# AssafSinger94/dino-tracker

Measured on AMD Instinct MI355X. Metric: query-points*frames/s, higher is better.
Workload: dtype mixed: fp16 ViT operands (one per value), f16 conv operands in Delta-DINO, f16 candidates + f32 deciders in the tracker; f32 accumulate; 1 GPU; 854x480x90 synthetic video (model res 854x476, 67x121 tokens, C=384), 1024 grid queries; 1 video(s) per step over 1 GPU(s); features=vit, mode=single, track_method=mfma, anchor_pairs=92091, correlation_maps_per_video=8380350, rccl_ranks=1, parallelism=video-parallel x1

## Files before the change

### dino_tracker_amd/_lib.py

```python
from __future__ import annotations

import ctypes
import os

_HERE = os.path.dirname(os.path.abspath(__file__))
LIB_PATH = os.path.join(_HERE, "csrc", "libdtk.so")

c_int, c_float, c_void_p, c_size_t = ctypes.c_int, ctypes.c_float, ctypes.c_void_p, ctypes.c_size_t


class Geom(ctypes.Structure):
    _fields_ = [("T", ctypes.c_int32), ("C", ctypes.c_int32), ("ph", ctypes.c_int32), ("pw", ctypes.c_int32),
                ("video_h", ctypes.c_int32), ("video_w", ctypes.c_int32), ("patch", ctypes.c_int32),
                ("stride", ctypes.c_int32), ("radius", ctypes.c_float)]

    @property
    def HW(self) -> int:
        return self.ph * self.pw


def make_geom(T: int, C: int, video_h: int, video_w: int, patch: int = 14, stride: int = 7, radius: float = 35.0) -> Geom:
    ph = 1 + (video_h - patch) // stride
    pw = 1 + (video_w - patch) // stride
    return Geom(T, C, ph, pw, video_h, video_w, patch, stride, radius)
# ... 81 lines not shown
    "dtk_profile_collect": (c_int, []),
    "dtk_profile_name": (ctypes.c_char_p, [c_int]),
    "dtk_profile_ms": (ctypes.c_double, [c_int]),
    "dtk_profile_launches": (ctypes.c_longlong, [c_int]),
    "dtk_pack_features": (c_int, [c_void_p, c_void_p, c_void_p, c_int, c_int, c_int, c_void_p]),
    "dtk_unpack_features": (c_int, [c_void_p, c_void_p, c_int, c_int, c_int, c_void_p]),
    "dtk_feature_norms": (c_int, [c_void_p, c_void_p, c_int, c_int, c_int, c_void_p]),
    "dtk_vit_workspace_bytes": (c_size_t, [ctypes.POINTER(VitModel), c_int, c_int, c_int]),
    "dtk_vit_forward": (c_int, [ctypes.POINTER(VitModel), c_void_p, c_int, c_int, c_int, c_void_p, c_void_p, c_void_p,
                                c_void_p, c_size_t, c_void_p]),
    "dtk_vit_attention": (c_int, [c_void_p, c_void_p, c_void_p, c_void_p, c_int, c_int, c_int, c_int, c_int, c_void_p]),
    "dtk_vit_attention_split": (c_int, [c_void_p] * 8 + [c_int, c_int, c_int, c_int, c_int, c_void_p]),
    "dtk_vit_gemm": (c_int, [ctypes.POINTER(VitGemmArgs), c_void_p]),
    "dtk_vit_gemm_split": (c_int, [ctypes.POINTER(VitGemmArgs), c_void_p]),
    "dtk_delta_dino_packed_floats": (c_size_t, [c_int, c_int]),
    "dtk_delta_dino_pack": (c_int, [c_int, c_int, c_void_p, c_void_p, c_void_p, c_void_p, c_void_p, c_void_p, c_float,
                                    c_void_p, c_void_p]),
    "dtk_delta_dino_workspace_bytes": (c_size_t, [ctypes.POINTER(Geom)]),
    "dtk_delta_dino_refine": (c_int, [ctypes.POINTER(Geom), c_void_p, c_void_p, ctypes.POINTER(c_void_p), c_void_p,
                                      c_void_p, c_int, c_int, c_void_p, c_size_t, c_void_p]),
    "dtk_delta_dino_refine_mode": (c_int, [ctypes.POINTER(Geom), c_void_p, c_void_p, ctypes.POINTER(c_void_p), c_void_p,
                                           c_void_p, c_int, c_int, c_int, c_void_p, c_size_t, c_void_p]),
    "dtk_sample_points": (c_int, [ctypes.POINTER(Geom), c_void_p, c_void_p, c_void_p, c_void_p, c_void_p, c_int, c_void_p]),
    "dtk_sample_grid": (c_int, [c_void_p, c_int, c_int, c_int, c_int, c_void_p, c_void_p, c_int, c_void_p]),
    "dtk_normalized_conv2d": (c_int, [c_void_p, c_void_p, c_void_p, c_void_p, c_int, c_int, c_int, c_int, c_int, c_int,
                                      c_void_p]),
    "dtk_corr_maps": (c_int, [ctypes.POINTER(Geom), c_void_p, c_void_p, c_void_p, c_void_p, c_void_p, c_void_p, c_void_p,
                              c_int, c_int, c_void_p]),
    "dtk_head_prepare": (c_int, [c_void_p, c_void_p, c_void_p, c_void_p, c_void_p, c_void_p]),
    "dtk_head_forward": (c_int, [ctypes.POINTER(Geom), c_void_p, c_void_p, c_void_p, c_int, c_int, c_void_p]),
    "dtk_head_forward_train": (c_int, [ctypes.POINTER(Geom), c_void_p, c_void_p, c_void_p, c_void_p, c_int, c_int, c_void_p]),
    "dtk_conv_split_weight_halves": (c_size_t, [c_int, c_int]),
    "dtk_conv_split_pack": (c_int, [c_void_p, c_int, c_int, c_int, c_void_p, c_void_p, c_void_p]),
    "dtk_conv_split_input": (c_int, [c_void_p, c_int, c_int, c_int, c_int, c_int, c_void_p, c_void_p, c_void_p, c_void_p]),
    "dtk_conv_split_run": (c_int, [c_void_p, c_void_p, c_void_p, c_void_p, c_void_p, c_int, c_int, c_int, c_int, c_int, c_int,
                                   c_int, c_int, c_void_p]),
    "dtk_conv_split_output": (c_int, [c_void_p, c_int, c_int, c_int, c_int, c_int, c_int, c_void_p, c_void_p, c_void_p]),
    "dtk_conv_wgrad_split_workspace_bytes": (c_size_t, [c_int, c_int, c_int, c_int, c_int, c_int]),
    "dtk_conv_wgrad_split": (c_int, [c_void_p, c_void_p, c_void_p, c_int, c_int, c_int, c_int, c_int, c_int, c_int, c_void_p,
                                     c_int, c_void_p, c_size_t, c_void_p]),
    "dtk_gemm_nt_f32_indexed": (c_int, [c_void_p, c_void_p, c_void_p, c_int, c_int, c_int, ctypes.c_int64, ctypes.c_int64,
                                        ctypes.c_int64, c_int, ctypes.c_int64, ctypes.c_int64, ctypes.c_int64, c_int, c_int,
                                        c_void_p, c_void_p, c_void_p, c_void_p, c_void_p]),
    "dtk_contrastive_workspace_bytes": (c_size_t, [c_int, c_int, c_int, c_int]),
    "dtk_contrastive_forward": (c_int, [c_void_p, c_void_p, c_void_p, ctypes.c_float, c_int, c_int, c_int, c_int, c_int, c_void_p,
                                        c_void_p, c_void_p, c_void_p, c_void_p, c_void_p]),
    "dtk_contrastive_backward": (c_int, [c_void_p, c_void_p, c_void_p, ctypes.c_float, c_int, c_int, c_int, c_int, c_int, c_void_p,
                                         c_void_p, c_void_p, c_void_p, c_void_p, c_void_p, c_void_p, c_void_p, c_size_t, c_void_p]),
    "dtk_emb_reg_forward": (c_int, [c_void_p, c_void_p, c_int, c_int, c_int, c_void_p, c_void_p, c_void_p]),
    "dtk_sample_bilinear_forward": (c_int, [c_void_p, c_void_p, c_void_p, ctypes.c_int32, ctypes.c_int32, ctypes.c_int32, ctypes.c_int32, ctypes.c_int32, c_void_p]),
    "dtk_sample_bilinear_backward": (c_int, [c_void_p, c_void_p, c_void_p, ctypes.c_int32, ctypes.c_int32, ctypes.c_int32, ctypes.c_int32, ctypes.c_int32, c_void_p]),
    "dtk_pow2_scale": (c_int, [c_void_p, ctypes.c_int64, c_void_p, c_void_p, c_void_p]),
    "dtk_adam_step": (c_int, [ctypes.POINTER(AdamArgs), c_void_p]),
    "dtk_adam_scalars": (c_int, [ctypes.POINTER(AdamArgs), ctypes.POINTER(ctypes.c_float)]),
    "dtk_adam_step_dev": (c_int, [ctypes.POINTER(AdamArgs), c_void_p, c_void_p]),
    "dtk_emb_reg_backward": (c_int, [c_void_p, c_void_p, c_void_p, c_void_p, c_int, c_int, c_int, c_void_p, c_void_p]),
    "dtk_corr_window_backward": (c_int, [ctypes.POINTER(Geom), c_void_p, c_void_p, c_void_p, c_void_p, c_void_p, c_void_p, c_void_p,
                                         c_void_p, c_void_p, c_int, c_void_p]),
    "dtk_head_backward": (c_int, [ctypes.POINTER(Geom), c_void_p, c_void_p, c_void_p, c_void_p, c_void_p, c_void_p, c_int, c_int,
                                  c_void_p]),
    "dtk_track_workspace_bytes": (c_size_t, [ctypes.POINTER(Geom), c_int, ctypes.POINTER(TrackOpts)]),
    "dtk_track": (c_int, [ctypes.POINTER(Geom), c_void_p, c_void_p, c_void_p, c_void_p, c_void_p, c_void_p, c_void_p,
                          c_void_p, c_void_p, c_int, c_void_p, ctypes.POINTER(TrackOpts), ctypes.POINTER(TrackStats),
                          c_void_p, c_size_t, c_void_p]),
    "dtk_argmax_cells": (c_int, [ctypes.POINTER(Geom), c_void_p, c_void_p, c_void_p, c_void_p, c_void_p, c_void_p, c_void_p,
                                 c_void_p, c_int, c_int, c_void_p, c_size_t, c_void_p]),
    "dtk_bb_nms_workspace_bytes": (c_size_t, [ctypes.POINTER(Geom), c_int]),
    "dtk_bb_nms": (c_int, [ctypes.POINTER(Geom), c_void_p, c_void_p, c_void_p, c_void_p, c_void_p, c_float, c_float, c_int,
                           c_void_p, c_void_p, c_int, c_void_p, c_size_t, c_void_p]),
    "dtk_traj_start_fg": (c_int, [c_void_p, c_int, c_int, c_void_p, c_int, c_int, c_int, c_void_p, c_void_p, c_void_p]),
    "dtk_nearest_traj_workspace_bytes": (c_size_t, [c_int, c_int, c_int, c_int]),
    "dtk_nearest_traj": (c_int, [c_void_p, c_int, c_int, c_int, c_int, c_float, c_float, c_void_p, c_void_p, c_size_t, c_void_p]),
    "dtk_of_filter_keep": (c_int, [c_void_p, c_int, c_int, c_void_p, c_int, c_int, c_float, c_float, c_void_p, c_void_p,
                                   c_void_p, c_void_p, c_int, c_void_p, c_void_p, c_void_p]),
    "dtk_feat_f16_bytes": (c_size_t, [ctypes.POINTER(Geom)]),
    "dtk_make_feat_f16": (c_int, [ctypes.POINTER(Geom), c_void_p, c_void_p, c_void_p, c_void_p]),
    "dtk_traj_cos_sims": (c_int, [c_void_p, c_void_p, c_void_p, c_int, c_int, c_int, c_void_p]),
    "dtk_build_anchor_sources": (c_int, [c_void_p, c_float, c_int, c_int, c_void_p, c_void_p, c_void_p, c_void_p,
                                         c_void_p, c_void_p, c_void_p, c_void_p, c_void_p]),
    "dtk_occlusion": (c_int, [c_void_p, c_void_p, c_void_p, c_void_p, c_void_p, c_float, c_float, c_void_p, c_int,
                              c_int, c_void_p]),
    "dtk_build_anchor_sources_needed": (c_int, [c_void_p, c_float, c_float, c_int, c_int, c_void_p, c_void_p, c_void_p,
                                                c_void_p, c_void_p, c_void_p, c_void_p, c_void_p, c_void_p]),
    "dtk_occlusion_needed": (c_int, [c_void_p, c_void_p, c_void_p, c_void_p, c_void_p, c_float, c_float, c_void_p, c_int,
                                     c_int, c_void_p]),
    "dtk_tapvid_counts": (c_int, [c_void_p, c_void_p, c_void_p, c_void_p, c_void_p, c_float, c_float, c_float, c_float,
                                  c_int, c_int, c_int, c_void_p, c_void_p]),
    "dtk_badja_counts": (c_int, [c_void_p, c_void_p, c_void_p, c_void_p, c_int, c_float, c_float, c_int, c_int, c_int, c_int, c_int,
                                 c_void_p, c_void_p, c_void_p]),
    "dtk_blurpool_forward": (c_int, [c_void_p, c_void_p, ctypes.c_int64, c_int, c_int, c_void_p]),
    "dtk_blurpool_backward": (c_int, [c_void_p, c_void_p, ctypes.c_int64, c_int, c_int, c_void_p]),
    "dtk_gemm_nt_f32": (c_int, [c_void_p, c_void_p, c_void_p, c_int, c_int, c_int, ctypes.c_int64, ctypes.c_int64, ctypes.c_int64,
                                c_int, ctypes.c_int64, ctypes.c_int64, ctypes.c_int64, c_int, c_int, c_void_p, c_void_p, c_void_p]),
    "dtk_im2col": (c_int, [c_void_p, c_void_p, c_int, c_int, c_int, c_int, c_int, c_int, c_int, c_int, c_int, c_int,
                           ctypes.c_int64, c_void_p]),
    "dtk_col2im": (c_int, [c_void_p, c_void_p, c_int, c_int, c_int, c_int, c_int, c_int, c_int, c_int, c_int, c_void_p]),
    "dtk_transpose_f32": (c_int, [c_void_p, c_void_p, ctypes.c_int64, ctypes.c_int64, c_int, c_void_p]),
    "dtk_resample2d_forward": (c_int, [c_void_p, c_void_p, ctypes.c_int64, c_int, c_int, c_int, c_int, c_void_p, c_void_p, c_void_p,
                                       c_void_p, c_void_p]),
    "dtk_resample2d_backward": (c_int, [c_void_p, c_void_p, ctypes.c_int64, c_int, c_int, c_int, c_int, c_void_p, c_void_p,
                                        c_void_p, c_void_p, c_void_p]),
    "dtk_batchnorm_workspace_bytes": (c_size_t, [c_int]),
    "dtk_batchnorm_train_forward": (c_int, [c_void_p, c_void_p, c_void_p, c_void_p, c_void_p, c_void_p, c_float, c_float,
                                            c_int, c_void_p, c_void_p, c_void_p, c_int, c_int, c_int, c_void_p, c_size_t,
                                            c_void_p]),
    "dtk_batchnorm_train_backward": (c_int, [c_void_p, c_void_p, c_void_p, c_void_p, c_void_p, c_void_p, c_int, c_void_p,
                                             c_void_p, c_void_p, c_void_p, c_int, c_int, c_int, c_void_p, c_size_t, c_void_p]),
    "dtk_pca_moments_workspace_bytes": (c_size_t, [ctypes.c_int64, c_int, ctypes.c_int64]),
    "dtk_pca_moments": (c_int, [c_void_p, ctypes.c_int64, c_int, c_int, ctypes.c_int64, c_void_p, c_void_p, c_void_p, c_size_t,
                                c_void_p]),
    "dtk_pca_project_workspace_bytes": (c_size_t, [ctypes.c_int64]),
    "dtk_pca_project": (c_int, [c_void_p, ctypes.c_int64, c_int, c_int, c_void_p, c_int, c_void_p, c_void_p, c_void_p, c_size_t,
                                c_void_p]),
    "dtk_fg_mask": (c_int, [c_void_p, c_int, c_int, c_void_p, c_float, c_int, c_int, c_int, c_int, c_int, c_int, c_void_p, c_void_p,
                            c_void_p]),
    "dtk_flow_pack": (c_int, [c_void_p, c_void_p, c_int, c_int, c_int, c_void_p]),
    "dtk_flow_cycle_masks": (c_int, [c_void_p, c_void_p, c_int, c_int, c_int, c_float, c_void_p, c_void_p]),
    "dtk_flow_traj_workspace_bytes": (c_size_t, [c_int, c_int, c_int]),
    "dtk_flow_traj_start": (c_int, [c_void_p, c_void_p, c_void_p, c_void_p, c_int, c_int, c_int, c_int, c_float, c_int, c_void_p,
                                    c_void_p, c_int, c_float, c_void_p, c_void_p, c_size_t, c_void_p]),
    "dtk_flow_traj_emit": (c_int, [c_int, c_int, c_int, c_int, c_int, c_int, c_void_p, c_void_p, c_void_p, c_size_t, c_void_p]),
    "dtk_render_prim_count": (ctypes.c_int64, [c_int, c_int, c_int, c_int]),
    "dtk_render_group_bytes": (c_size_t, [ctypes.c_int64, ctypes.c_int64, c_int, c_int, c_int]),
    "dtk_render_prims": (c_int, [c_void_p, c_void_p, c_void_p, c_void_p, c_int, c_int, c_int, c_int, c_int, c_int, c_int, c_int,
                                 c_float, c_float, c_int, c_void_p, c_void_p]),
    "dtk_render_pred_gt_prims": (c_int, [c_void_p, c_void_p, c_void_p, c_void_p, c_void_p, c_int, c_int, c_int, c_int, c_int,
                                         c_int, c_int, c_void_p, c_void_p]),
    "dtk_render_tile_counts": (c_int, [c_void_p, ctypes.c_int64, c_int, c_int, c_int, c_void_p, c_void_p]),
    "dtk_render_tile_keys": (c_int, [c_void_p, c_void_p, ctypes.c_int64, c_int, c_int, c_int, ctypes.c_int64, c_void_p, c_void_p]),
    "dtk_render_blend": (c_int, [c_void_p, c_void_p, ctypes.c_int64, c_void_p, ctypes.c_int64, c_void_p, c_int, c_int, c_int,
                                 c_void_p, c_void_p, c_void_p]),
    "dtk_resize_workspace_bytes": (c_size_t, [c_int, c_int, c_int, c_int, c_int, c_int, c_int, c_int]),
    "dtk_resize_u8": (c_int, [c_void_p, c_int, c_int, c_int, c_int, c_int, c_int, c_void_p, c_void_p, c_int, c_void_p, c_void_p, c_int,
                              c_void_p, c_int, c_int, c_void_p, c_void_p, c_size_t, c_void_p]),
    "dtk_raft_conv_packed_halves": (c_size_t, [c_int, c_int, c_int, c_int]),
    "dtk_raft_conv_pack": (c_int, [c_void_p, c_int, c_int, c_int, c_int, c_float, c_void_p, c_void_p, c_void_p]),
    "dtk_raft_conv": (c_int, [ctypes.POINTER(RaftConvArgs), c_void_p]),
    "dtk_raft_instance_norm_workspace_bytes": (c_size_t, [c_int, c_int, c_int, c_int]),
    "dtk_raft_instance_norm": (c_int, [c_void_p, c_void_p, c_void_p, c_int, c_int, c_int, c_int, c_float, c_int, c_void_p, c_size_t,
                                       c_void_p]),
    "dtk_raft_pyramid_floats": (c_size_t, [c_int, c_int, c_int]),
    "dtk_raft_corr_pyramid": (c_int, [c_void_p, c_void_p, c_int, c_int, c_int, c_int, c_int, c_void_p, c_void_p]),
    "dtk_raft_lookup": (c_int, [c_void_p, c_void_p, ctypes.c_int64, c_int, c_int, c_int, c_void_p, ctypes.c_int64, c_void_p]),
    "dtk_raft_upsample": (c_int, [c_void_p, ctypes.c_int64, c_void_p, c_int, c_int, c_int, c_void_p, c_void_p]),
    "dtk_raft_workspace_bytes": (c_size_t, [c_int, c_int, c_int]),
    "dtk_raft_forward": (c_int, [ctypes.POINTER(RaftModel), c_void_p, c_void_p, c_int, c_int, c_int, c_int, c_int, c_void_p, c_void_p,
                                 c_size_t, c_void_p]),
}

_LIB = None


def lib() -> ctypes.CDLL:
    global _LIB
    if _LIB is None:
        if not os.path.isfile(LIB_PATH):
            raise RuntimeError(
                f"{LIB_PATH} is missing: build the HIP extension first (python -c 'import __graft_entry__ as g; "
                "g.build()' or make -C dino_tracker_amd/csrc). There is no CPU fallback for the hot path.")
        handle = ctypes.CDLL(LIB_PATH)
        for name, (res, args) in SIGNATURES.items():
            fn = getattr(handle, name)
            fn.restype = res
            fn.argtypes = args
        _LIB = handle
    return _LIB


# ... 4 lines not shown
```

### dino_tracker_amd/csrc/anchors.hip

```cpp
#include "common.h"

namespace {

__device__ __forceinline__ bool is_anchor(const float* cs, float th, int n, int T, int t) {
    return cs[(size_t)n * T + t] >= th;
}

__device__ __forceinline__ bool is_undecided(float c, float anchor_th, float cos_th) { return !(c >= anchor_th) && !(c < cos_th); }
__device__ __forceinline__ bool is_needed(float c, float anchor_th, float cos_th) { return c >= anchor_th || !(c < cos_th); }

__global__ __launch_bounds__(256) void query_need_kernel(const float* __restrict__ cs, float anchor_th, float cos_th, int N, int T,
                                                         int32_t* __restrict__ n_anchors, int32_t* __restrict__ need_w) {
    const int n = blockIdx.x * blockDim.x + threadIdx.x;
    if (n >= N) return;
    int anchors = 0, undecided = 0, needed = 0;
    for (int t = 0; t < T; ++t) {
        const float c = cs[(size_t)n * T + t];
        anchors += c >= anchor_th ? 1 : 0;
        undecided += is_undecided(c, anchor_th, cos_th) ? 1 : 0;
        needed += is_needed(c, anchor_th, cos_th) ? 1 : 0;
    }
    n_anchors[n] = anchors;
    need_w[n] = (anchors > 0 && undecided > 0) ? needed : 0;
}
// ... 89 lines not shown
}

__global__ void finalize_counts_kernel(const int32_t* __restrict__ pair_off, int N, int T, int32_t* __restrict__ counts) {
    if (threadIdx.x == 0 && blockIdx.x == 0) {
        counts[0] = pair_off[N];
        counts[1] = pair_off[N] * T;
    }
}

__global__ __launch_bounds__(256) void emit_sources_kernel(const float* __restrict__ cs, float th, int N, int T,
                                                           const int32_t* __restrict__ pair_off,
                                                           const int32_t* __restrict__ frame_off,
                                                           int32_t* __restrict__ pair_frame,
                                                           int32_t* __restrict__ src_row, int32_t* __restrict__ tgt,
                                                           int32_t* __restrict__ out_idx) {
    __shared__ int lds4[4];
    const int a = blockIdx.x;
    int carry = frame_off[a];
    for (int n0 = 0; n0 < N; n0 += 256) {
        const int n = n0 + threadIdx.x;
        const int flag = (n < N && is_anchor(cs, th, n, T, a)) ? 1 : 0;
        int total;
        const int incl = block_scan_incl(flag, lds4, &total);
        if (flag) {
            const int j = carry + incl - 1;
            int rank = 0;
            for (int t = 0; t < a; ++t) rank += is_anchor(cs, th, n, T, t) ? 1 : 0;
            const int p = pair_off[n] + rank;
            pair_frame[p] = a;
            const size_t mb = (size_t)j * T;
            for (int t = 0; t < T; ++t) {
                src_row[mb + t] = n * T + t;
                tgt[mb + t] = a;
                out_idx[mb + t] = p * T + t;
            }
        }
        carry += total;
    }
}

__global__ __launch_bounds__(256) void emit_needed_sources_kernel(const float* __restrict__ cs, float anchor_th, float cos_th,
                                                                  int N, int T, const int32_t* __restrict__ pair_off,
                                                                  const int32_t* __restrict__ frame_off,
                                                                  const int32_t* __restrict__ need_w,
                                                                  int32_t* __restrict__ pair_frame,
                                                                  int32_t* __restrict__ src_row, int32_t* __restrict__ tgt,
                                                                  int32_t* __restrict__ out_idx) {
    __shared__ int lds4[4];
    const int a = blockIdx.x;
    int carry = frame_off[a];
    for (int n0 = 0; n0 < N; n0 += 256) {
        const int n = n0 + threadIdx.x;
        const bool anchor = n < N && is_anchor(cs, anchor_th, n, T, a);
        const int weight = anchor ? need_w[n] : 0;
        int total;
        const int incl = block_scan_incl(weight, lds4, &total);
        if (anchor) {
            int rank = 0;
            for (int t = 0; t < a; ++t) rank += is_anchor(cs, anchor_th, n, T, t) ? 1 : 0;
            const int p = pair_off[n] + rank;
            pair_frame[p] = a;
            if (weight > 0) {
                int m = carry + incl - weight;
                for (int t = 0; t < T; ++t) {
                    if (!is_needed(cs[(size_t)n * T + t], anchor_th, cos_th)) continue;
                    src_row[m] = n * T + t;
                    tgt[m] = a;
                    out_idx[m] = p * T + t;
                    ++m;
                }
            }
        }
        carry += total;
    }
}

__device__ __forceinline__ float anchor_dist(const float* __restrict__ green, const float* __restrict__ tr, int p, int a,
                                             int T, int t) {
    const float dx = green[((size_t)p * T + t) * 2] - tr[2 * a];
    const float dy = green[((size_t)p * T + t) * 2 + 1] - tr[2 * a + 1];
    return sqrtf(__fadd_rn(__fmul_rn(dx, dx), __fmul_rn(dy, dy)));
}

template <bool PRUNED>
__global__ __launch_bounds__(256) void occlusion_kernel(const float* __restrict__ green,
                                                        const int32_t* __restrict__ pair_off,
                                                        const int32_t* __restrict__ pair_frame,
                                                        const float* __restrict__ traj, const float* __restrict__ cs,
                                                        float anchor_th, float cos_th, uint8_t* __restrict__ occ, int N,
                                                        int T) {
    extern __shared__ float smem_occ[];
    float* med = smem_occ;
    __shared__ float red[4];
    const int n = blockIdx.x;
    const int lane = threadIdx.x & 63, w = threadIdx.x >> 6;
    float* d = smem_occ + T + w * T;
    const int p0 = pair_off[n], A = pair_off[n + 1] - p0;
    const float* tr = traj + (size_t)n * T * 2;
    if (A <= 0) {
        for (int t = threadIdx.x; t < T; t += 256) occ[(size_t)n * T + t] = 1;
        return;
    }
    if constexpr (PRUNED) {
        int undecided = 0;
        for (int t = threadIdx.x; t < T; t += 256) undecided |= is_undecided(cs[(size_t)n * T + t], anchor_th, cos_th) ? 1 : 0;
        if (!__syncthreads_or(undecided)) {
            for (int t = threadIdx.x; t < T; t += 256) occ[(size_t)n * T + t] = cs[(size_t)n * T + t] < cos_th ? 1 : 0;
            return;
        }
    }
    const int want = (A - 1) / 2;
    for (int t = w; t < T; t += 4) {
        if constexpr (PRUNED)
            if (!is_needed(cs[(size_t)n * T + t], anchor_th, cos_th)) continue;
        for (int k = lane; k < A; k += WAVE) d[k] = anchor_dist(green, tr, p0 + k, pair_frame[p0 + k], T, t);
        __builtin_amdgcn_fence(__ATOMIC_RELEASE, "wavefront");
        __builtin_amdgcn_wave_barrier();
        for (int k = lane; k < A; k += WAVE) {
            const float dk = d[k];
            int rank = 0;
            for (int k2 = 0; k2 < A; ++k2) {
                const float d2 = d[k2];
                rank += (d2 < dk || (d2 == dk && k2 < k)) ? 1 : 0;
            }
            if (rank == want) med[t] = dk;
        }
        __builtin_amdgcn_fence(__ATOMIC_RELEASE, "wavefront");
        __builtin_amdgcn_wave_barrier();
    }
    __syncthreads();
    float tau = -INFINITY;
    for (int t = threadIdx.x; t < T; t += 256)
        if (cs[(size_t)n * T + t] >= anchor_th) tau = fmaxf(tau, med[t]);
    tau = wave_max(tau);
    if (lane == 0) red[w] = tau;
    __syncthreads();
    tau = fmaxf(fmaxf(red[0], red[1]), fmaxf(red[2], red[3]));
    for (int t = threadIdx.x; t < T; t += 256) {
        const float c = cs[(size_t)n * T + t];
        const bool far = (!PRUNED || is_needed(c, anchor_th, cos_th)) && med[t] > tau;
        occ[(size_t)n * T + t] = (far || c < cos_th) ? 1 : 0;
    }
}

}

extern "C" int dtk_build_anchor_sources(const float* cs, float anchor_th, int N, int T, int32_t* n_anchors,
                                        int32_t* pair_off, int32_t* pair_frame, int32_t* src_row, int32_t* tgt,
                                        int32_t* out_idx, int32_t* counts, int32_t* scratch, void* stream) {
    DTK_REQUIRE(cs && n_anchors && pair_off && pair_frame && src_row && tgt && out_idx && counts && scratch,
                "dtk_build_anchor_sources: null pointer");
    DTK_REQUIRE(N > 0 && T > 0 && (long long)N * T * T < 2147483647LL, "dtk_build_anchor_sources: N*T*T out of range");
    hipStream_t st = dtk_stream(stream);
    int32_t* frame_cnt = scratch;
    int32_t* frame_off = scratch + T;
    DTK_LAUNCH("anchor_count", anchor_count_kernel, dim3(dtk_cdiv(N, 256)), dim3(256), 0, st, cs, anchor_th, N, T, n_anchors);
    DTK_LAUNCH("exclusive_scan", exclusive_scan_kernel, dim3(1), dim3(256), 0, st, n_anchors, pair_off, N, counts + 2);
    DTK_LAUNCH("frame_count", frame_count_kernel, dim3(T), dim3(256), 0, st, cs, anchor_th, N, T, frame_cnt);
    DTK_LAUNCH("exclusive_scan", exclusive_scan_kernel, dim3(1), dim3(256), 0, st, frame_cnt, frame_off, T, (int32_t*)nullptr);
    DTK_LAUNCH("finalize_counts", finalize_counts_kernel, dim3(1), dim3(64), 0, st, pair_off, N, T, counts);
    DTK_LAUNCH("emit_sources", emit_sources_kernel, dim3(T), dim3(256), 0, st, cs, anchor_th, N, T, pair_off, frame_off,
                       pair_frame, src_row, tgt, out_idx);
    return DTK_OK;
}

extern "C" int dtk_occlusion(const float* green, const int32_t* pair_off, const int32_t* pair_frame, const float* traj,
                             const float* cs, float anchor_th, float cos_th, uint8_t* occ, int N, int T, void* stream) {
    DTK_REQUIRE(green && pair_off && pair_frame && traj && cs && occ && N >= 0 && T > 0, "dtk_occlusion: bad args");
    DTK_REQUIRE((size_t)5 * T * sizeof(float) <= 60 * 1024, "dtk_occlusion: T=%d too large", T);
    if (N == 0) return DTK_OK;
    DTK_LAUNCH("occlusion", occlusion_kernel<false>, dim3(N), dim3(256), (size_t)5 * T * sizeof(float), dtk_stream(stream), green,
                       pair_off, pair_frame, traj, cs, anchor_th, cos_th, occ, N, T);
    return DTK_OK;
}

extern "C" int dtk_build_anchor_sources_needed(const float* cs, float anchor_th, float cos_th, int N, int T, int32_t* n_anchors,
                                               int32_t* pair_off, int32_t* pair_frame, int32_t* src_row, int32_t* tgt,
                                               int32_t* out_idx, int32_t* counts, int32_t* scratch, void* stream) {
    DTK_REQUIRE(cs && n_anchors && pair_off && pair_frame && src_row && tgt && out_idx && counts && scratch,
                "dtk_build_anchor_sources_needed: null pointer");
    DTK_REQUIRE(N > 0 && T > 0 && (long long)N * T * T < 2147483647LL, "dtk_build_anchor_sources_needed: N*T*T out of range");
    hipStream_t st = dtk_stream(stream);
    int32_t* frame_cnt = scratch;
    int32_t* frame_off = scratch + T;
    int32_t* need_w = scratch + 2 * T + 2;
    DTK_LAUNCH("query_need", query_need_kernel, dim3(dtk_cdiv(N, 256)), dim3(256), 0, st, cs, anchor_th, cos_th, N, T, n_anchors,
               need_w);
    DTK_LAUNCH("exclusive_scan", exclusive_scan_kernel, dim3(1), dim3(256), 0, st, n_anchors, pair_off, N, counts + 2);
    DTK_LAUNCH("frame_weight", frame_weight_kernel, dim3(T), dim3(256), 0, st, cs, anchor_th, N, T, need_w, frame_cnt);
    DTK_LAUNCH("exclusive_scan", exclusive_scan_kernel, dim3(1), dim3(256), 0, st, frame_cnt, frame_off, T, (int32_t*)nullptr);
    DTK_LAUNCH("finalize_counts", finalize_needed_counts_kernel, dim3(1), dim3(256), 0, st, pair_off, frame_off, need_w, N, T,
               counts);
    DTK_LAUNCH("emit_sources", emit_needed_sources_kernel, dim3(T), dim3(256), 0, st, cs, anchor_th, cos_th, N, T, pair_off,
               frame_off, need_w, pair_frame, src_row, tgt, out_idx);
    return DTK_OK;
}

extern "C" int dtk_occlusion_needed(const float* green, const int32_t* pair_off, const int32_t* pair_frame, const float* traj,
                                    const float* cs, float anchor_th, float cos_th, uint8_t* occ, int N, int T, void* stream) {
    DTK_REQUIRE(green && pair_off && pair_frame && traj && cs && occ && N >= 0 && T > 0, "dtk_occlusion_needed: bad args");
    DTK_REQUIRE((size_t)5 * T * sizeof(float) <= 60 * 1024, "dtk_occlusion_needed: T=%d too large", T);
    if (N == 0) return DTK_OK;
    DTK_LAUNCH("occlusion", occlusion_kernel<true>, dim3(N), dim3(256), (size_t)5 * T * sizeof(float), dtk_stream(stream), green,
                       pair_off, pair_frame, traj, cs, anchor_th, cos_th, occ, N, T);
    return DTK_OK;
}


__global__ __launch_bounds__(256) void tapvid_counts_kernel(const float* __restrict__ pred, const uint8_t* __restrict__ pred_occ,
                                                            const float* __restrict__ gt, const uint8_t* __restrict__ gt_occ,
                                                            const int32_t* __restrict__ qframe, float spx, float spy,
                                                            float sgx, float sgy, int first_mode, int N, int T,
                                                            unsigned long long* __restrict__ counts) {
    const long long i = (long long)blockIdx.x * 256 + threadIdx.x;
    int c[18];
#pragma unroll
    for (int k = 0; k < 18; ++k) c[k] = 0;
    if (i < (long long)N * T) {
        const int n = (int)(i / T), t = (int)(i - (long long)n * T);
        const int qf = qframe[n];
        const bool ev = first_mode ? (t > qf) : (t != qf);
        if (ev) {
            const bool vis = gt_occ[i] == 0, pvis = pred_occ[i] == 0;
            const float dx = __fsub_rn(__fmul_rn(pred[2 * i], spx), __fmul_rn(gt[2 * i], sgx));
            const float dy = __fsub_rn(__fmul_rn(pred[2 * i + 1], spy), __fmul_rn(gt[2 * i + 1], sgy));
            const float d2 = __fadd_rn(__fmul_rn(dx, dx), __fmul_rn(dy, dy));
            c[0] = 1;
            c[1] = (pvis == vis);
            c[2] = vis;
#pragma unroll
            for (int k = 0; k < 5; ++k) {
                const float th = (float)(1 << k);
                const bool within = d2 < th * th;
                c[3 + 3 * k] = within && vis;
                c[4 + 3 * k] = within && vis && pvis;
                c[5 + 3 * k] = ((!vis) && pvis) || ((!within) && pvis);
            }
        }
    }
#pragma unroll
    for (int k = 0; k < 18; ++k) {
        const int s = wave_sum_i(c[k]);
        if ((threadIdx.x & 63) == 0 && s) atomicAdd(&counts[k], (unsigned long long)s);
    }
}

extern "C" int dtk_tapvid_counts(const float* pred_tracks, const uint8_t* pred_occluded, const float* gt_tracks,
                                 const uint8_t* gt_occluded, const int32_t* query_frame, float pred_scale_x,
                                 float pred_scale_y, float gt_scale_x, float gt_scale_y, int first_mode, int N, int T,
                                 unsigned long long* counts18, void* stream) {
    DTK_REQUIRE(counts18, "dtk_tapvid_counts: null pointer");
    DTK_REQUIRE(N >= 0 && T > 0, "dtk_tapvid_counts: bad sizes");
    hipStream_t st = dtk_stream(stream);
    DTK_HIP(hipMemsetAsync(counts18, 0, 18 * sizeof(unsigned long long), st));
    if (N == 0) return DTK_OK;
    DTK_REQUIRE(pred_tracks && pred_occluded && gt_tracks && gt_occluded && query_frame, "dtk_tapvid_counts: null pointer");
    DTK_LAUNCH("tapvid_counts", tapvid_counts_kernel, dim3(dtk_cdiv((long long)N * T, 256)), dim3(256), 0, st, pred_tracks,
               pred_occluded, gt_tracks, gt_occluded, query_frame, pred_scale_x, pred_scale_y, gt_scale_x, gt_scale_y,
               first_mode, N, T, counts18);
    return DTK_OK;
}


template <typename M>
__global__ __launch_bounds__(256) void badja_area_kernel(const M* __restrict__ seg, long long HW,
                                                         unsigned long long* __restrict__ areas) {
    const M* frame = seg + (size_t)blockIdx.y * HW;
    int c = 0;
    for (long long p = (long long)blockIdx.x * 256 + threadIdx.x; p < HW; p += (long long)gridDim.x * 256) c += frame[p] > (M)0;
    c = wave_sum_i(c);
    if ((threadIdx.x & 63) == 0 && c) atomicAdd(&areas[blockIdx.y], (unsigned long long)c);
}

__global__ __launch_bounds__(256) void badja_counts_kernel(const float* __restrict__ pred, const double* __restrict__ gt,
                                                           const uint8_t* __restrict__ gt_occ,
                                                           const unsigned long long* __restrict__ areas, float spx, float spy,
                                                           int N, int T, int T_seg, unsigned long long* __restrict__ counts) {
    const long long idx = (long long)blockIdx.x * 256 + threadIdx.x;
    const int per = T_seg - 1;
    int vis = 0, in_seg = 0, in_3px = 0;
    if (idx < (long long)N * per) {
        const int n = (int)(idx / per), t = 1 + (int)(idx - (long long)n * per);
        const size_t at = (size_t)n * T + t;
        if (gt_occ[at] == 0) {
            const float thr = __fmul_rn(0.2f, __fsqrt_rn((float)areas[t]));
            const double dx = __dsub_rn((double)__fmul_rn(pred[2 * at], spx), gt[2 * at]);
            const double dy = __dsub_rn((double)__fmul_rn(pred[2 * at + 1], spy), gt[2 * at + 1]);
// ... 43 lines not shown
```

### dino_tracker_amd/csrc/track_exact.hip

```cpp
#include <limits.h>
#include "common.h"
#include "head_common.h"

namespace {

constexpr int TM = 64, TN = 64, TK = 16;
constexpr int HR = 6;
constexpr int HR_LARGE = 2;

__global__ void head_prepare_kernel(const float* __restrict__ w1, const float* __restrict__ b1,
                                    const float* __restrict__ w2, const float* __restrict__ b2,
                                    float* __restrict__ head) {
    const int ch = threadIdx.x;
    if (ch >= DTK_HEAD_HIDDEN) return;
    float s1 = 0.f, s2 = 0.f;
    for (int t = 0; t < 9; ++t) {
        s1 += w1[ch * 9 + t];
        s2 += w2[ch * 9 + t];
    }
    auto fix = [](float s) {
        if (fabsf(s) < 1e-8f) s = (s > 0.f ? 1.f : (s < 0.f ? -1.f : 0.f)) * 1e-8f;
        return s;
    };
    s1 = fix(s1);
    s2 = fix(s2);
    for (int t = 0; t < 9; ++t) {
        head[ch * 9 + t] = w1[ch * 9 + t] / s1;
        head[144 + 16 + ch * 9 + t] = w2[ch * 9 + t] / s2;
    }
    head[144 + ch] = b1[ch];
    if (ch == 0) head[144 + 16 + 144] = b2[0];
}

__global__ __launch_bounds__(256) void row_norms_kernel(const float* __restrict__ emb,
                                                        const int32_t* __restrict__ src_row,
                                                        float* __restrict__ snorm, int m0, int count, int M,
                                                        const int32_t* __restrict__ dM, int C) {
    const int i = blockIdx.x * 4 + (threadIdx.x >> 6);
    if (i >= count) return;
    const int lane = threadIdx.x & 63;
    const int m = m0 + i;
    float s = 0.f;
    if (m < dtk_active(M, dM)) {
        const float* p = emb + (size_t)(src_row ? src_row[m] : m) * C;
        for (int c = lane * 4; c < C; c += 256) {
            const float4 v = *reinterpret_cast<const float4*>(p + c);
            s += v.x * v.x + v.y * v.y + v.z * v.z + v.w * v.w;
        }
        s = wave_sum(s);
    }
    if (lane == 0) snorm[i] = sqrtf(s);
}

__global__ __launch_bounds__(256) void corr_exact_kernel(dtk_geom g, const float* __restrict__ feat,
                                                         const float* __restrict__ norms,
                                                         const float* __restrict__ emb,
                                                         const int32_t* __restrict__ src_row,
                                                         const int32_t* __restrict__ tgt,
                                                         const float* __restrict__ snorm, float* __restrict__ maps,
                                                         int m0, int count, int M, const int32_t* __restrict__ dM,
                                                         int HWs, int relu) {
    __shared__ __attribute__((aligned(16))) float As[TK][TM + 4];
    __shared__ __attribute__((aligned(16))) float Bs[TK][TN + 4];
    __shared__ int s_tgt[TM];
    __shared__ int s_row[TM];
    __shared__ int s_fr[2];
    const int HW = g.ph * g.pw;
    const int active = min(dtk_active(M, dM), m0 + count);
    const int tile_m0 = m0 + blockIdx.y * TM;
    if (tile_m0 >= active) return;
    const int cell0 = blockIdx.x * TN;
    const int tid = threadIdx.x;
    if (tid < TM) {
        const int m = tile_m0 + tid;
        const bool ok = m < active;
        int f = ok ? tgt[m] : -1;
        if (ok) f = min(max(f, 0), g.T - 1);
        s_tgt[tid] = f;
        s_row[tid] = ok ? (src_row ? src_row[m] : m) : (src_row ? src_row[tile_m0] : tile_m0);
        int lo = ok ? f : INT_MAX, hi = f;
#pragma unroll
        for (int o = 32; o > 0; o >>= 1) {
            lo = min(lo, __shfl_xor(lo, o, WAVE));
            hi = max(hi, __shfl_xor(hi, o, WAVE));
        }
        if (tid == 0) {
            s_fr[0] = lo;
            s_fr[1] = hi;
        }
    }
    __syncthreads();
    const int fmin = s_fr[0], fmax = s_fr[1];
    const int ty = tid >> 4, tx = tid & 15;
    const int lr = tid >> 2, lk = (tid & 3) * 4;
    const float* arow = emb + (size_t)s_row[lr] * g.C;
    const int lcell = cell0 + lr;
    for (int f = fmin; f <= fmax; ++f) {
        bool mine = false;
#pragma unroll
        for (int i = 0; i < 4; ++i) mine |= (s_tgt[ty * 4 + i] == f);
        if (!__syncthreads_or(mine)) continue;
        const float* brow = feat + ((size_t)f * HW + min(lcell, HW - 1)) * g.C;
        float acc[4][4];
#pragma unroll
        for (int i = 0; i < 4; ++i)
#pragma unroll
            for (int j = 0; j < 4; ++j) acc[i][j] = 0.f;
        for (int k0 = 0; k0 < g.C; k0 += TK) {
            float4 a = make_float4(0.f, 0.f, 0.f, 0.f), b = a;
            if (k0 + lk < g.C) {
                a = *reinterpret_cast<const float4*>(arow + k0 + lk);
                if (lcell < HW) b = *reinterpret_cast<const float4*>(brow + k0 + lk);
            }
            As[lk + 0][lr] = a.x; As[lk + 1][lr] = a.y; As[lk + 2][lr] = a.z; As[lk + 3][lr] = a.w;
            Bs[lk + 0][lr] = b.x; Bs[lk + 1][lr] = b.y; Bs[lk + 2][lr] = b.z; Bs[lk + 3][lr] = b.w;
            __syncthreads();
#pragma unroll
            for (int kk = 0; kk < TK; ++kk) {
                const float4 av = *reinterpret_cast<const float4*>(&As[kk][ty * 4]);
                const float4 bv = *reinterpret_cast<const float4*>(&Bs[kk][tx * 4]);
                const float aa[4] = {av.x, av.y, av.z, av.w}, bb[4] = {bv.x, bv.y, bv.z, bv.w};
#pragma unroll
                for (int i = 0; i < 4; ++i)
#pragma unroll
                    for (int j = 0; j < 4; ++j) acc[i][j] = fmaf(aa[i], bb[j], acc[i][j]);
            }
            __syncthreads();
        }
#pragma unroll
        for (int i = 0; i < 4; ++i) {
            const int r = ty * 4 + i;
            if (s_tgt[r] != f) continue;
            const int ml = tile_m0 - m0 + r;
            const float sn = snorm[ml];
#pragma unroll
            for (int j = 0; j < 4; ++j) {
                const int cell = cell0 + tx * 4 + j;
                if (cell < HW) {
                    const float den = fmaxf(sn * norms[(size_t)f * HW + cell], 1e-8f);
                    const float rho = acc[i][j] / den;
                    maps[(size_t)ml * HWs + cell] = relu ? fmaxf(rho, 0.f) : rho;
                }
            }
        }
    }
}

__device__ __forceinline__ float block_max(float v, float* red) {
    v = wave_max(v);
    __syncthreads();
    if ((threadIdx.x & 63) == 0) red[threadIdx.x >> 6] = v;
    __syncthreads();
    return fmaxf(fmaxf(red[0], red[1]), fmaxf(red[2], red[3]));
}
__device__ __forceinline__ float block_sum(float v, float* red) {
    v = wave_sum(v);
    __syncthreads();
    if ((threadIdx.x & 63) == 0) red[threadIdx.x >> 6] = v;
    __syncthreads();
    return (red[0] + red[1]) + (red[2] + red[3]);
}

}

namespace {

template <bool LARGE>
__global__ __launch_bounds__(256) void head_exact_kernel(dtk_geom g, const float* __restrict__ head,
                                                         const float* __restrict__ maps, int HWs,
                                                         const int32_t* __restrict__ out_idx,
                                                         float* __restrict__ out_xy, int m0, int count, int M,
                                                         const int32_t* __restrict__ dM, int normalized,
                                                         float* __restrict__ stats) {
    extern __shared__ __attribute__((aligned(16))) float smem[];
    const int HW = g.ph * g.pw, pw = g.pw, ph = g.ph;
    const int HWp = (HW + 3) & ~3;
    constexpr int HRK = LARGE ? HR_LARGE : HR;
    float* sz = LARGE ? smem : smem + HWp;
    float* sh = sz + HWp;
    float* red = sh + DTK_HEAD_HIDDEN * (HRK + 2) * pw;
    int* redi = reinterpret_cast<int*>(red + 8);
    const int i = blockIdx.x;
    const int m = m0 + i;
    if (i >= count || m >= dtk_active(M, dM)) return;
    const int tid = threadIdx.x;
    const float* map = maps + (size_t)i * HWs;
    const float* sx = map;
    if constexpr (!LARGE) {
        for (int c = tid; c < HW; c += 256) smem[c] = map[c];
        sx = smem;
    }
    __syncthreads();

    float best = -1.f;
    int bi = INT_MAX;
    for (int c = tid; c < HW; c += 256) {
        const float v = sx[c];
        if (v > best) { best = v; bi = c; }
    }
#pragma unroll
    for (int o = 32; o > 0; o >>= 1) {
        const float ov = __shfl_xor(best, o, WAVE);
        const int oi = __shfl_xor(bi, o, WAVE);
        if (ov > best || (ov == best && oi < bi)) { best = ov; bi = oi; }
    }
    if ((tid & 63) == 0) { red[tid >> 6] = best; redi[tid >> 6] = bi; }
    __syncthreads();
    best = red[0]; bi = redi[0];
#pragma unroll
    for (int w = 1; w < 4; ++w)
        if (red[w] > best || (red[w] == best && redi[w] < bi)) { best = red[w]; bi = redi[w]; }
    const int kstar = bi;
    __syncthreads();

    const float* w1 = head;
    const float* b1 = head + 144;
    const float* w2 = head + 160;
    const float b2 = head[304];
    const int ring = HRK + 2;
    for (int r0 = 0; r0 < ph; r0 += HRK) {
        const int nout = min(HRK, ph - r0);
        for (int idx = tid; idx < (nout + 2) * pw; idx += 256) {
            const int hr = idx / pw, c = idx - hr * pw;
// ... 81 lines not shown
    for (int o = 32; o > 0; o >>= 1) {
        const float ov = __shfl_xor(best, o, WAVE);
        const int oi = __shfl_xor(bi, o, WAVE);
        if (ov > best || (ov == best && oi < bi)) { best = ov; bi = oi; }
    }
    if ((tid & 63) == 0) { red[tid >> 6] = best; redi[tid >> 6] = bi; }
    __syncthreads();
    if (tid == 0) {
        best = red[0]; bi = redi[0];
        for (int w = 1; w < 4; ++w)
            if (red[w] > best || (red[w] == best && redi[w] < bi)) { best = red[w]; bi = redi[w]; }
        const int oi = out_idx ? out_idx[m0 + i] : m0 + i;
        arg_cell[oi] = bi;
        arg_cos[oi] = best;
    }
}

extern "C" int dtk_head_prepare(const float* w1, const float* b1, const float* w2, const float* b2, float* head,
                                void* stream) {
    DTK_REQUIRE(w1 && b1 && w2 && b2 && head, "dtk_head_prepare: null pointer");
    DTK_LAUNCH("head_prepare", head_prepare_kernel, dim3(1), dim3(64), 0, dtk_stream(stream), w1, b1, w2, b2, head);
    return DTK_OK;
}

extern "C" int dtk_head_forward(const dtk_geom* g, const float* head, const float* maps, float* out_xy, int B,
                                int normalized, void* stream);

static inline int exact_hws(const dtk_geom* g) { return (g->ph * g->pw + 63) & ~63; }
static inline size_t exact_head_lds(const dtk_geom* g, bool large) {
    const int HWp = (g->ph * g->pw + 3) & ~3;
    return sizeof(float) * (size_t)((large ? 1 : 2) * HWp + DTK_HEAD_HIDDEN * ((large ? HR_LARGE : HR) + 2) * g->pw + 16);
}
constexpr size_t EXACT_LDS_MAX = 160 * 1024;
static int launch_head_exact(const char* who, const char* name, const dtk_geom* g, const float* head, const float* maps, int HWs,
                             const int32_t* out_idx, float* out_xy, int m0, int cnt, int M, const int32_t* dM, int normalized,
                             float* stats, hipStream_t st) {
    const bool large = exact_head_lds(g, false) > EXACT_LDS_MAX;
    const size_t lds = exact_head_lds(g, large);
    DTK_REQUIRE(lds <= EXACT_LDS_MAX, "%s: token grid %dx%d needs %zu B of LDS (> 160 KiB)", who, g->ph, g->pw, lds);
    if (large) {
        DTK_HIP(hipFuncSetAttribute(reinterpret_cast<const void*>(head_exact_kernel<true>),
                                    hipFuncAttributeMaxDynamicSharedMemorySize, (int)lds));
        DTK_LAUNCH(name, head_exact_kernel<true>, dim3(cnt), dim3(256), lds, st, *g, head, maps, HWs, out_idx, out_xy, m0, cnt, M,
                   dM, normalized, stats);
    } else {
        DTK_HIP(hipFuncSetAttribute(reinterpret_cast<const void*>(head_exact_kernel<false>),
                                    hipFuncAttributeMaxDynamicSharedMemorySize, (int)lds));
        DTK_LAUNCH(name, head_exact_kernel<false>, dim3(cnt), dim3(256), lds, st, *g, head, maps, HWs, out_idx, out_xy, m0, cnt, M,
                   dM, normalized, stats);
    }
    return DTK_OK;
}
bool dtk_track_exact_fits(const dtk_geom* g) { return exact_head_lds(g, true) <= EXACT_LDS_MAX; }
constexpr int EXACT_CHUNK = 4096;

size_t dtk_track_exact_workspace_bytes(const dtk_geom* g, int M) {
    const int chunk = M < EXACT_CHUNK ? (M < 64 ? 64 : M) : EXACT_CHUNK;
    return (size_t)chunk * (exact_hws(g) + 1) * sizeof(float);
}

int dtk_track_exact(const dtk_geom* g, const float* feat, const float* norms, const float* head, const float* emb,
                    const int32_t* src_row, const int32_t* tgt, const int32_t* out_idx, float* out_xy, int M,
                    const int32_t* dM, int normalized, void* workspace, size_t workspace_bytes, void* stream) {
    DTK_REQUIRE(g->C % TK == 0, "dtk_track(exact): C=%d must be a multiple of %d", g->C, TK);
    const int HWs = exact_hws(g);
    DTK_REQUIRE(dtk_track_exact_fits(g), "dtk_track(exact): token grid %dx%d needs %zu B of LDS (> 160 KiB)", g->ph, g->pw,
                exact_head_lds(g, true));
    long long chunk = (long long)(workspace_bytes / ((size_t)(HWs + 1) * sizeof(float)));
    if (chunk > M) chunk = M;
    if (chunk > 65535LL * TM) chunk = 65535LL * TM;
    if (chunk < 1) {
        dtk_set_error("dtk_track(exact): workspace of %zu B holds no map (need %zu B per source)", workspace_bytes,
                      (size_t)(HWs + 1) * sizeof(float));
        return DTK_E_WORKSPACE;
    }
    hipStream_t st = dtk_stream(stream);
    float* maps = reinterpret_cast<float*>(workspace);
    float* snorm = maps + (size_t)chunk * HWs;
    const int HW = g->ph * g->pw;
    for (long long m0 = 0; m0 < M; m0 += chunk) {
        const int cnt = (int)((M - m0) < chunk ? (M - m0) : chunk);
        DTK_LAUNCH("row_norms", row_norms_kernel, dim3(dtk_cdiv(cnt, 4)), dim3(256), 0, st, emb, src_row, snorm, (int)m0,
                           cnt, M, dM, g->C);
        DTK_LAUNCH("corr_exact", corr_exact_kernel, dim3(dtk_cdiv(HW, TN), dtk_cdiv(cnt, TM)), dim3(256), 0, st, *g, feat,
                           norms, emb, src_row, tgt, snorm, maps, (int)m0, cnt, M, dM, HWs, 1);
        const int rc = launch_head_exact("dtk_track(exact)", "head_exact", g, head, maps, HWs, out_idx, out_xy, (int)m0, cnt, M, dM,
                                         normalized, nullptr, st);
        if (rc) return rc;
    }
    return DTK_OK;
}

extern "C" int dtk_head_forward(const dtk_geom* g, const float* head, const float* maps, float* out_xy, int B,
                                int normalized, void* stream) {
    DTK_REQUIRE(g && head && maps && out_xy && B >= 0, "dtk_head_forward: null pointer");
    DTK_REQUIRE(g->ph > 0 && g->pw > 0 && g->stride > 0 && g->patch > 0, "dtk_head_forward: bad geometry");
    if (B == 0) return DTK_OK;
    return launch_head_exact("dtk_head_forward", "head_exact", g, head, maps, g->ph * g->pw, nullptr, out_xy, 0, B, B, nullptr,
                             normalized, nullptr, dtk_stream(stream));
}

namespace {

constexpr int HB_RD = 5, HB_WX = 2 * HB_RD + 5, HB_WH = 2 * HB_RD + 3, HB_WZ = 2 * HB_RD + 1;

__global__ __launch_bounds__(256) void head_backward_kernel(dtk_geom g, const float* __restrict__ head,
                                                            const float* __restrict__ maps, const float* __restrict__ stats,
                                                            const float* __restrict__ gout, float* __restrict__ dmaps,
                                                            float* __restrict__ dhead, int B, int normalized) {
    constexpr int NH = HB_WH * HB_WH, NZ = HB_WZ * HB_WZ, XP = HB_WX + 1;
    __shared__ float s_x[4][HB_WX * XP];
    __shared__ float s_h[4][DTK_HEAD_HIDDEN * NH];
    __shared__ unsigned char s_m[4][DTK_HEAD_HIDDEN * NH];
    __shared__ float s_z[4][NZ], s_dz[4][NZ];
    const int lane = threadIdx.x & 63, w = threadIdx.x >> 6;
    const int b = blockIdx.x * 4 + w;
    if (b >= B) return;
    const int ph = g.ph, pw = g.pw, HW = ph * pw;
    const float* st = stats + 4 * (size_t)b;
    const int kstar = __float_as_int(st[0]);
    const float zmax = st[1], Z = st[2];
    const int kr = kstar / pw, kc = kstar % pw;
    const float* map = maps + (size_t)b * HW;
    const float* w1 = head;
    const float* b1 = head + 144;
    const float* w2 = head + 160;
    const float b2 = head[304];
    float* sx = s_x[w];
    float* sh = s_h[w];
    unsigned char* sm = s_m[w];
    float* sz = s_z[w];
    float* sdz = s_dz[w];
    auto wsync = [] {
        __builtin_amdgcn_fence(__ATOMIC_RELEASE, "wavefront");
        __builtin_amdgcn_wave_barrier();
        __builtin_amdgcn_fence(__ATOMIC_ACQUIRE, "wavefront");
    };
    for (int i = lane; i < HB_WX * HB_WX; i += WAVE) {
        const int jr = i / HB_WX, jc = i - jr * HB_WX;
        const int r = kr - (HB_RD + 2) + jr, c = kc - (HB_RD + 2) + jc;
        sx[jr * XP + jc] = (r >= 0 && r < ph && c >= 0 && c < pw) ? map[r * pw + c] : 0.f;
    }
    wsync();
    for (int i = lane; i < NH; i += WAVE) {
        const int hy = i / HB_WH, hx = i - hy * HB_WH;
        const int r = kr - (HB_RD + 1) + hy, c = kc - (HB_RD + 1) + hx;
        const bool in = r >= 0 && r < ph && c >= 0 && c < pw;
        float x9[9];
#pragma unroll
        for (int dy = 0; dy < 3; ++dy)
#pragma unroll
            for (int dx = 0; dx < 3; ++dx) x9[dy * 3 + dx] = sx[(hy + dy) * XP + hx + dx];
#pragma unroll
        for (int ch = 0; ch < DTK_HEAD_HIDDEN; ++ch) {
            float a = 0.f;
#pragma unroll
            for (int t = 0; t < 9; ++t) a = fmaf(w1[ch * 9 + t], x9[t], a);
            a += b1[ch];
            const bool pos = in && a > 0.f;
            sh[ch * NH + i] = pos ? a : 0.f;
            sm[ch * NH + i] = pos ? 1 : 0;
        }
    }
    wsync();
    for (int i = lane; i < NZ; i += WAVE) {
        const int zy = i / HB_WZ, zx = i - zy * HB_WZ;
        float a = 0.f;
// ... 151 lines not shown
    const float* fbase = feat + (size_t)f * HW * C;
    float* dbase = dfeat + (size_t)f * HW * C;
    const float* mp = maps + (size_t)b * HW;
    const float* dm = dmaps + (size_t)b * HW;
    const int r0 = max(kr - (HB_RD + 2), 0), r1 = min(kr + (HB_RD + 2), ph - 1);
    const int c0 = max(kc - (HB_RD + 2), 0), c1 = min(kc + (HB_RD + 2), pw - 1);
    for (int r = r0 + w; r <= r1; r += 4)
        for (int c = c0; c <= c1; ++c) {
            const int cell = r * pw + c;
            const float gk = dm[cell], rho = mp[cell];
            if (gk == 0.f || !(rho > 0.f)) continue;
            const float fn = norms[(size_t)f * HW + cell];
            const float den = sn * fn;
            const bool clamped = !(den > 1e-8f);
            const float inv_den = clamped ? 1e8f : 1.f / den;
            const float a_s = clamped ? 0.f : rho * inv_ss;
            const float a_f = clamped ? 0.f : rho / (fn * fn);
            const float* fp = fbase + (size_t)cell * C;
            float* dp = dbase + (size_t)cell * C;
#pragma unroll
            for (int j = 0; j < MAXJ; ++j) {
                const int ch = j * WAVE + lane;
                if (j < nj && ch < C) {
                    const float fv = fp[ch];
                    ds[j] += gk * (fv * inv_den - a_s * s[j]);
                    atomicAdd(dp + ch, gk * (s[j] * inv_den - a_f * fv));
                }
            }
        }
#pragma unroll
    for (int j = 0; j < MAXJ; ++j) s_ds[w][j * WAVE + lane] = ds[j];
    __syncthreads();
    for (int c = threadIdx.x; c < C; c += 256) demb[(size_t)b * C + c] = (s_ds[0][c] + s_ds[1][c]) + (s_ds[2][c] + s_ds[3][c]);
}

}

extern "C" int dtk_corr_window_backward(const dtk_geom* g, const float* feat, const float* norms, const float* emb,
                                        const int32_t* tgt, const float* maps, const float* dmaps, const float* stats,
                                        float* demb, float* dfeat, int B, void* stream) {
    DTK_REQUIRE(g && feat && norms && emb && tgt && maps && dmaps && stats && demb && dfeat && B >= 0,
                "dtk_corr_window_backward: null pointer");
    DTK_REQUIRE(g->C > 0 && g->C <= 1024, "dtk_corr_window_backward: C=%d outside 1..1024", g->C);
    DTK_REQUIRE(g->radius / (float)g->stride <= (float)HB_RD, "dtk_corr_window_backward: radius / stride > %d", HB_RD);
    if (B == 0) return DTK_OK;
    DTK_LAUNCH("train_corr_bwd", corr_window_backward_kernel, dim3(B), dim3(256), 0, dtk_stream(stream), *g, feat,
               norms, emb, tgt, maps, dmaps, stats, demb, dfeat, B);
    return DTK_OK;
}

extern "C" int dtk_head_forward_train(const dtk_geom* g, const float* head, const float* maps, float* out_xy, float* stats, int B,
                                      int normalized, void* stream) {
    DTK_REQUIRE(g && head && maps && out_xy && stats && B >= 0, "dtk_head_forward_train: null pointer");
    DTK_REQUIRE(g->ph > 0 && g->pw > 0 && g->stride > 0 && g->patch > 0, "dtk_head_forward_train: bad geometry");
    if (B == 0) return DTK_OK;
    return launch_head_exact("dtk_head_forward_train", "train_head_fwd", g, head, maps, g->ph * g->pw, nullptr, out_xy, 0, B, B,
                             nullptr, normalized, stats, dtk_stream(stream));
}

extern "C" int dtk_head_backward(const dtk_geom* g, const float* head, const float* maps, const float* stats, const float* grad_out,
                                 float* dmaps, float* dhead_partial, int B, int normalized, void* stream) {
    DTK_REQUIRE(g && head && maps && stats && grad_out && dmaps && dhead_partial && B >= 0, "dtk_head_backward: null pointer");
    DTK_REQUIRE(g->stride > 0 && g->radius / (float)g->stride <= (float)HB_RD,
                "dtk_head_backward: disk radius %g px exceeds %d cells of stride %d", (double)g->radius, HB_RD, g->stride);
    if (B == 0) return DTK_OK;
    DTK_LAUNCH("train_head_bwd", head_backward_kernel, dim3(dtk_cdiv(B, 4)), dim3(256), 0, dtk_stream(stream), *g, head, maps,
               stats, grad_out, dmaps, dhead_partial, B, normalized);
    return DTK_OK;
}

extern "C" int dtk_corr_maps(const dtk_geom* g, const float* feat, const float* norms, const float* emb,
                             const int32_t* src_row, const int32_t* tgt, float* maps, float* snorm_scratch, int M,
                             int relu, void* stream) {
    DTK_REQUIRE(g && feat && norms && emb && tgt && maps && snorm_scratch, "dtk_corr_maps: null pointer");
    DTK_REQUIRE(g->T > 0 && g->ph > 0 && g->pw > 0 && g->C > 0 && g->C % TK == 0, "dtk_corr_maps: bad geometry (C %% %d)", TK);
    DTK_REQUIRE(M >= 0, "dtk_corr_maps: negative M");
    const int HW = g->ph * g->pw;
    hipStream_t st = dtk_stream(stream);
    const long long step = 65535LL * TM;
    for (long long m0 = 0; m0 < M; m0 += step) {
        const int cnt = (int)((M - m0) < step ? (M - m0) : step);
        DTK_LAUNCH("row_norms", row_norms_kernel, dim3(dtk_cdiv(cnt, 4)), dim3(256), 0, st, emb, src_row, snorm_scratch + m0,
                   (int)m0, cnt, M, (const int32_t*)nullptr, g->C);
        DTK_LAUNCH("corr_exact", corr_exact_kernel, dim3(dtk_cdiv(HW, TN), dtk_cdiv(cnt, TM)), dim3(256), 0, st, *g, feat,
                   norms, emb, src_row, tgt, snorm_scratch + m0, maps + (size_t)m0 * HW, (int)m0, cnt, M,
                   (const int32_t*)nullptr, HW, relu);
    }
    return DTK_OK;
}

int dtk_argmax_exact(const dtk_geom* g, const float* feat, const float* norms, const float* emb, const int32_t* src_row,
                     const int32_t* tgt, const int32_t* out_idx, int32_t* arg_cell, float* arg_cos, int M, void* workspace,
                     size_t workspace_bytes, void* stream) {
    DTK_REQUIRE(g->C % TK == 0, "dtk_argmax_cells(exact): C=%d must be a multiple of %d", g->C, TK);
    const int HWs = exact_hws(g), HW = g->ph * g->pw;
    long long chunk = (long long)(workspace_bytes / ((size_t)(HWs + 1) * sizeof(float)));
    if (chunk > M) chunk = M;
    if (chunk > 65535LL * TM) chunk = 65535LL * TM;
    if (chunk < 1) {
        dtk_set_error("dtk_argmax_cells(exact): workspace of %zu B holds no map", workspace_bytes);
        return DTK_E_WORKSPACE;
    }
    hipStream_t st = dtk_stream(stream);
    float* maps = reinterpret_cast<float*>(workspace);
    float* snorm = maps + (size_t)chunk * HWs;
    for (long long m0 = 0; m0 < M; m0 += chunk) {
        const int cnt = (int)((M - m0) < chunk ? (M - m0) : chunk);
        DTK_LAUNCH("row_norms", row_norms_kernel, dim3(dtk_cdiv(cnt, 4)), dim3(256), 0, st, emb, src_row, snorm, (int)m0, cnt, M,
                   (const int32_t*)nullptr, g->C);
        DTK_LAUNCH("corr_exact", corr_exact_kernel, dim3(dtk_cdiv(HW, TN), dtk_cdiv(cnt, TM)), dim3(256), 0, st, *g, feat, norms,
                   emb, src_row, tgt, snorm, maps, (int)m0, cnt, M, (const int32_t*)nullptr, HWs, 0);
        DTK_LAUNCH("argmax_exact", argmax_exact_kernel, dim3(cnt), dim3(256), 0, st, maps, HW, HWs, out_idx, arg_cell, arg_cos,
                   (int)m0, cnt);
    }
    return DTK_OK;
}

namespace {

constexpr int NMS_VPT = 40;

__device__ __forceinline__ unsigned order_key(float v) {
    const unsigned b = __float_as_uint(v);
    return (b & 0x80000000u) ? ~b : (b | 0x80000000u);
}

__global__ __launch_bounds__(256) void bb_nms_kernel(dtk_geom g, const float* __restrict__ maps, int HWs, float box_half,
                                                     float iou_thresh, int topk, float* __restrict__ peak_affs,
                                                     float* __restrict__ r_out, int m0, int count) {
    __shared__ float red[4];
    __shared__ int redi[4];
    __shared__ int s_cnt;
    const int i = blockIdx.x;
    if (i >= count) return;
    const int tid = threadIdx.x, HW = g.ph * g.pw;
    const float* map = maps + (size_t)i * HWs;
    float v[NMS_VPT];
    float best = -INFINITY;
    int bi = INT_MAX;
#pragma unroll
    for (int j = 0; j < NMS_VPT; ++j) {
        const int c = tid + 256 * j;
        v[j] = c < HW ? map[c] : -INFINITY;
        if (c < HW && v[j] > best) { best = v[j]; bi = c; }
    }
#pragma unroll
    for (int o = 32; o > 0; o >>= 1) {
        const float ov = __shfl_xor(best, o, WAVE);
        const int oi = __shfl_xor(bi, o, WAVE);
        if (ov > best || (ov == best && oi < bi)) { best = ov; bi = oi; }
    }
    if ((tid & 63) == 0) { red[tid >> 6] = best; redi[tid >> 6] = bi; }
    __syncthreads();
    best = red[0]; bi = redi[0];
#pragma unroll
    for (int w = 1; w < 4; ++w)
        if (red[w] > best || (red[w] == best && redi[w] < bi)) { best = red[w]; bi = redi[w]; }
    unsigned K = 0;
    for (int bit = 31; bit >= 0; --bit) {
        const unsigned cand = K | (1u << bit);
        int c = 0;
#pragma unroll
        for (int j = 0; j < NMS_VPT; ++j) c += (tid + 256 * j < HW && order_key(v[j]) >= cand) ? 1 : 0;
        c = wave_sum_i(c);
        __syncthreads();
        if (tid == 0) s_cnt = 0;
        __syncthreads();
        if ((tid & 63) == 0) atomicAdd(&s_cnt, c);
        __syncthreads();
        if (s_cnt >= topk) K = cand;
    }
    const float half = (float)(g.patch / 2), st = (float)g.stride;
    const float pcx = half + st * (float)(bi % g.pw), pcy = half + st * (float)(bi / g.pw);
    const float px1 = pcx - box_half, px2 = pcx + box_half, py1 = pcy - box_half, py2 = pcy + box_half;
    const float parea = (px2 - px1) * (py2 - py1);
    float b = -INFINITY;
    int nsupp = 0;
#pragma unroll
    for (int j = 0; j < NMS_VPT; ++j) {
        const int c = tid + 256 * j;
        if (c < HW && c != bi && order_key(v[j]) >= K) {
            const float cx = half + st * (float)(c % g.pw), cy = half + st * (float)(c / g.pw);
            const float x1 = cx - box_half, x2 = cx + box_half, y1 = cy - box_half, y2 = cy + box_half;
            const float iw = fmaxf(fminf(x2, px2) - fmaxf(x1, px1), 0.f), ih = fmaxf(fminf(y2, py2) - fmaxf(y1, py1), 0.f);
            const float inter = iw * ih;
            const float iou = inter / (parea + (x2 - x1) * (y2 - y1) - inter);
            if (iou > iou_thresh) ++nsupp;
            else b = fmaxf(b, v[j]);
        }
    }
    b = wave_max(b);
    nsupp = wave_sum_i(nsupp);
    __syncthreads();
    if ((tid & 63) == 0) { red[tid >> 6] = b; redi[tid >> 6] = nsupp; }
    __syncthreads();
    if (tid == 0) {
        b = fmaxf(fmaxf(red[0], red[1]), fmaxf(red[2], red[3]));
        nsupp = redi[0] + redi[1] + redi[2] + redi[3];
        float c4[4] = {best, b, nsupp >= 1 ? 0.f : -INFINITY, nsupp >= 2 ? 0.f : -INFINITY};
        float t1 = -INFINITY, t2 = -INFINITY;
#pragma unroll
        for (int q = 0; q < 4; ++q) {
            if (c4[q] > t1) { t2 = t1; t1 = c4[q]; }
            else if (c4[q] > t2) t2 = c4[q];
        }
        peak_affs[2 * (size_t)(m0 + i)] = t1;
        peak_affs[2 * (size_t)(m0 + i) + 1] = t2;
        r_out[m0 + i] = t2 / t1;
    }
}

}

extern "C" size_t dtk_bb_nms_workspace_bytes(const dtk_geom* g, int M) { return dtk_track_exact_workspace_bytes(g, M); }

extern "C" int dtk_bb_nms(const dtk_geom* g, const float* feat, const float* norms, const float* emb, const int32_t* src_row,
                          const int32_t* tgt, float box_size, float iou_thresh, int topk, float* peak_affs, float* r, int M,
                          void* workspace, size_t workspace_bytes, void* stream) {
    DTK_REQUIRE(g && feat && norms && emb && tgt && peak_affs && r && workspace, "dtk_bb_nms: null pointer");
    DTK_REQUIRE(M >= 0, "dtk_bb_nms: negative M");
    if (M == 0) return DTK_OK;
    DTK_REQUIRE(g->C % TK == 0, "dtk_bb_nms: C=%d must be a multiple of %d", g->C, TK);
    const int HWs = exact_hws(g), HW = g->ph * g->pw;
    DTK_REQUIRE(HW <= 256 * NMS_VPT, "dtk_bb_nms: %d cells per frame (max %d)", HW, 256 * NMS_VPT);
    DTK_REQUIRE(topk >= 2 && topk <= HW, "dtk_bb_nms: topk=%d must be in [2, %d] (torch.topk)", topk, HW);
    long long chunk = (long long)(workspace_bytes / ((size_t)(HWs + 1) * sizeof(float)));
    if (chunk > M) chunk = M;
    if (chunk > 65535LL * TM) chunk = 65535LL * TM;
    if (chunk < 1) {
        dtk_set_error("dtk_bb_nms: workspace of %zu B holds no map", workspace_bytes);
        return DTK_E_WORKSPACE;
    }
    hipStream_t st = dtk_stream(stream);
    float* maps = reinterpret_cast<float*>(workspace);
    float* snorm = maps + (size_t)chunk * HWs;
    for (long long m0 = 0; m0 < M; m0 += chunk) {
        const int cnt = (int)((M - m0) < chunk ? (M - m0) : chunk);
        DTK_LAUNCH("row_norms", row_norms_kernel, dim3(dtk_cdiv(cnt, 4)), dim3(256), 0, st, emb, src_row, snorm, (int)m0, cnt, M,
                   (const int32_t*)nullptr, g->C);
        DTK_LAUNCH("corr_exact", corr_exact_kernel, dim3(dtk_cdiv(HW, TN), dtk_cdiv(cnt, TM)), dim3(256), 0, st, *g, feat, norms,
                   emb, src_row, tgt, snorm, maps, (int)m0, cnt, M, (const int32_t*)nullptr, HWs, 0);
        DTK_LAUNCH("bb_nms", bb_nms_kernel, dim3(cnt), dim3(256), 0, st, *g, maps, HWs, box_size, iou_thresh, topk, peak_affs, r,
                   (int)m0, cnt);
    }
    return DTK_OK;
}
```

### dino_tracker_amd/csrc/track_mfma.hip

```cpp
#include <limits.h>
#include <stdlib.h>
#include <type_traits>
#include "common.h"
#include "head_common.h"

int dtk_track_exact(const dtk_geom* g, const float* feat, const float* norms, const float* head, const float* emb,
                    const int32_t* src_row, const int32_t* tgt, const int32_t* out_idx, float* out_xy, int M,
                    const int32_t* dM, int normalized, void* workspace, size_t workspace_bytes, void* stream);
size_t dtk_track_exact_workspace_bytes(const dtk_geom* g, int M);
bool dtk_track_exact_fits(const dtk_geom* g);

namespace {

typedef _Float16 half_t;
typedef _Float16 h2 __attribute__((ext_vector_type(2)));
typedef _Float16 h8 __attribute__((ext_vector_type(8)));
typedef float f4 __attribute__((ext_vector_type(4)));

constexpr float FSCALE = 32.f;
constexpr float INV_SCALE2 = 1.f / 1024.f;
constexpr float EPS_C = 3e-3f;
constexpr int KC = 10;
constexpr int CM = 64, CN = 128, CK = 32;
constexpr int NB_MAX = 1024;
constexpr int RD = 5;
constexpr int MFMA_CHUNK = 16384;
constexpr int MFMA_SUPER = 4194304;

struct Rec {
    float amax;
    int ncand;
    int cand[KC];
    float zmax, Z;
};

__host__ __device__ inline int pw_pad(int pw) { return (pw + CN - 1) / CN * CN; }
__host__ __device__ inline int map_xw(int pw) { return pw_pad(pw) + 16; }
__host__ __device__ inline int hw_pad(int ph, int pw) { return ph * pw_pad(pw); }

__global__ __launch_bounds__(256) void feat16_kernel(const float* __restrict__ feat, const float* __restrict__ norms,
                                                     half_t* __restrict__ f16, int T, int ph, int pw, int PWP, int C) {
    const long long cell = (long long)blockIdx.x * 4 + (threadIdx.x >> 6);
    const int HWp = ph * PWP, HW = ph * pw;
    if (cell >= (long long)T * HWp) return;
    const int lane = threadIdx.x & 63;
    const int t = (int)(cell / HWp), pc = (int)(cell % HWp);
    const int r = pc / PWP, c = pc - r * PWP;
    half_t* o = f16 + cell * C;
    if (c >= pw) {
        for (int k = lane * 8; k < C; k += 512) *reinterpret_cast<uint4*>(o + k) = make_uint4(0, 0, 0, 0);
        return;
    }
    const float* p = feat + ((size_t)t * HW + r * pw + c) * C;
    const float nrm = norms[(size_t)t * HW + r * pw + c];
    const float sc = nrm > 1e-30f ? FSCALE / nrm : 0.f;
    for (int k = lane * 8; k < C; k += 512) {
        const float4 a = *reinterpret_cast<const float4*>(p + k), b = *reinterpret_cast<const float4*>(p + k + 4);
        h8 v = {(half_t)(a.x * sc), (half_t)(a.y * sc), (half_t)(a.z * sc), (half_t)(a.w * sc),
                (half_t)(b.x * sc), (half_t)(b.y * sc), (half_t)(b.z * sc), (half_t)(b.w * sc)};
        *reinterpret_cast<h8*>(o + k) = v;
    }
}

__host__ __device__ inline bool peaks_wide_ok(int C) { return C == 768 || C == 1024; }

constexpr float RC_SCALE_MAX = 32.f;
__host__ __device__ inline size_t split_planes_offset(const dtk_geom* g) {
    return ((size_t)g->T * hw_pad(g->ph, g->pw) * g->C * 2 + 255) / 256 * 256;
}
__host__ __device__ inline bool has_split_planes(const dtk_geom* g) {
    return g->C == 384 && (long long)g->T * g->ph * g->pw * g->C * 4 < (1LL << 32);
}
__host__ __device__ inline size_t rc_scale_offset(const dtk_geom* g) {
    const size_t unit = (size_t)g->T * hw_pad(g->ph, g->pw) * g->C * 2;
    const size_t end = has_split_planes(g) ? split_planes_offset(g) + (size_t)g->T * g->ph * g->pw * g->C * 4 : unit;
    return (end + 255) / 256 * 256;
}
__global__ __launch_bounds__(256) void rcscale_max_kernel(const float* __restrict__ norms, long long n, unsigned* __restrict__ slot) {
    float m = 0.f;
    for (long long i = (long long)blockIdx.x * 256 + threadIdx.x; i < n; i += (long long)gridDim.x * 256) {
        const float v = norms[i];
        m = fmaxf(m, v == v ? v : 3.0e38f);
    }
    m = wave_max(m);
    if ((threadIdx.x & 63) == 0) atomicMax(slot + 1, __float_as_uint(m));
}
__global__ void rcscale_final_kernel(unsigned* __restrict__ slot) {
    const float m = __uint_as_float(slot[1]);
    float sc = RC_SCALE_MAX;
    while (sc > 0x1p-40f && m * sc > 16384.f) sc *= 0.5f;
    reinterpret_cast<float*>(slot)[0] = sc;
}
__global__ __launch_bounds__(256) void featsplit_kernel(const float* __restrict__ feat, half_t* __restrict__ fs,
                                                        long long n8, const float* __restrict__ rc_scale) {
    const long long i = (long long)blockIdx.x * 256 + threadIdx.x;
    if (i >= n8) return;
    const float RC_SCALE = *rc_scale;
    const float4 a = *reinterpret_cast<const float4*>(feat + i * 8), b = *reinterpret_cast<const float4*>(feat + i * 8 + 4);
    const float x[8] = {a.x, a.y, a.z, a.w, b.x, b.y, b.z, b.w};
    h8 hi, lo;
#pragma unroll
    for (int e = 0; e < 8; ++e) {
        const float xs = x[e] * RC_SCALE;
        hi[e] = (half_t)xs;
        lo[e] = (half_t)(xs - (float)hi[e]);
    }
    const long long chunk = i >> 2;
    const int piece = (int)(i & 3);
    *reinterpret_cast<h8*>(fs + chunk * 64 + piece * 8) = hi;
    *reinterpret_cast<h8*>(fs + chunk * 64 + 32 + piece * 8) = lo;
}

__global__ __launch_bounds__(256) void src16_kernel(const float* __restrict__ emb, const int32_t* __restrict__ src_row,
                                                    half_t* __restrict__ s16, int m0, int count, int M,
                                                    const int32_t* __restrict__ dM, int C, float scale,
                                                    float* __restrict__ rown) {
    const int i = blockIdx.x * 4 + (threadIdx.x >> 6);
    if (i >= count) return;
    const int lane = threadIdx.x & 63;
    const int m = m0 + i;
    half_t* o = s16 + (size_t)i * C;
    if (m >= dtk_active(M, dM)) {
        for (int k = lane * 8; k < C; k += 512) *reinterpret_cast<uint4*>(o + k) = make_uint4(0, 0, 0, 0);
        return;
    }
    const float* p = emb + (size_t)(src_row ? src_row[m] : m) * C;
    float s = 0.f;
    for (int k = lane * 4; k < C; k += 256) {
        const float4 v = *reinterpret_cast<const float4*>(p + k);
        s += v.x * v.x + v.y * v.y + v.z * v.z + v.w * v.w;
    }
    s = sqrtf(wave_sum(s));
    if (rown && lane == 0) rown[i] = s;
    const float sc = s > 1e-30f ? scale / s : 0.f;
    for (int k = lane * 8; k < C; k += 512) {
        const float4 a = *reinterpret_cast<const float4*>(p + k), b = *reinterpret_cast<const float4*>(p + k + 4);
        h8 v = {(half_t)(a.x * sc), (half_t)(a.y * sc), (half_t)(a.z * sc), (half_t)(a.w * sc),
                (half_t)(b.x * sc), (half_t)(b.y * sc), (half_t)(b.z * sc), (half_t)(b.w * sc)};
        *reinterpret_cast<h8*>(o + k) = v;
    }
}

__device__ __forceinline__ int swz(int row, int piece) {
    const int f = (0x1230 >> (((row >> 2) & 3) * 4)) & 3;
    return row * 4 + (piece ^ f);
}

struct TileRec {
    float v1, v2;
    uint32_t idx;
};

template <bool PEAKS>
__global__ __launch_bounds__(256) void corr16_tiled_kernel(dtk_geom g, const half_t* __restrict__ f16,
                                                     const half_t* __restrict__ s16, const int32_t* __restrict__ tgt,
                                                     half_t* __restrict__ maps, TileRec* __restrict__ trec, int m0,
                                                     int count, int M, const int32_t* __restrict__ dM, int HWp, int MP,
                                                     int dbg) {
    __shared__ uint4 smem_ab[2 * (CM + CN) * 4];
    uint4 (*As)[CM * 4] = reinterpret_cast<uint4 (*)[CM * 4]>(smem_ab);
    uint4 (*Bs)[CN * 4] = reinterpret_cast<uint4 (*)[CN * 4]>(smem_ab + 2 * CM * 4);
    half_t* Ts = reinterpret_cast<half_t*>(smem_ab);
    constexpr int TP16 = CN + 8;
    __shared__ int s_tgt[CM];
    __shared__ int s_fr[2];
    const int active = min(dtk_active(M, dM), m0 + count);
    const int NT = HWp / CN, MT = (count + CM - 1) / CM;
    int bx, by;
    {
        const int L = blockIdx.x, xcd = L & 7, k = L >> 3;
        const int mt_per = (MT + 7) >> 3;
        const int per_panel = mt_per * 8;
        const int p = k / per_panel, rem = k - p * per_panel;
        by = (rem >> 3) * 8 + xcd;
        bx = p * 8 + (rem & 7);
        if (by >= MT || bx >= NT) return;
    }
    const int tile_m0 = m0 + by * CM;
    if (tile_m0 >= active) return;
    const int cell0 = bx * CN;
    const int tid = threadIdx.x, lane = tid & 63, w = tid >> 6;
    if (tid < CM) {
        const int m = tile_m0 + tid;
        const bool ok = m < active;
        int f = ok ? min(max(tgt[m], 0), g.T - 1) : -1;
        s_tgt[tid] = f;
        int lo = ok ? f : INT_MAX, hi = f;
#pragma unroll
        for (int o = 32; o > 0; o >>= 1) {
            lo = min(lo, __shfl_xor(lo, o, WAVE));
            hi = max(hi, __shfl_xor(hi, o, WAVE));
        }
        if (tid == 0) { s_fr[0] = lo; s_fr[1] = hi; }
// ... 1606 lines not shown
            redo.out_idx[slot] = oi;
        } else {
            out_xy[2 * (size_t)oi] = s_out[w][0];
            out_xy[2 * (size_t)oi + 1] = s_out[w][1];
        }
    }
}

struct MfmaLayout {
    size_t s16, maps, rec, wpk, kstar, xwin, snorm, rown, perm, hist, off, cursor, bsum, nvalid, redo_cnt, redo_lists, exact, total;
    int HWk, nkeys, nblocks, cap;
    size_t unc_lists, trec;
    int MP;
    int chunk;
    int super;
    int HWp;
};

MfmaLayout mfma_layout(const dtk_geom* g, int M, int round_sources) {
    MfmaLayout L;
    L.chunk = M < MFMA_CHUNK ? ((M + CM - 1) / CM * CM) : MFMA_CHUNK;
    const int round = round_sources > 0 ? (round_sources + 255) / 256 * 256 : MFMA_SUPER;
    L.super = M < round ? ((M + CM - 1) / CM * CM) : round;
    if (L.chunk > L.super) L.chunk = L.super;
    L.HWp = hw_pad(g->ph, g->pw);
    auto al = [](size_t x) { return (x + 255) & ~(size_t)255; };
    size_t off = 0;
    L.s16 = off; off = al(off + (size_t)L.super * g->C * 2);
    L.MP = ((g->ph + 2) * map_xw(g->pw) + 32 + 7) & ~7;
    L.maps = off; off = al(off + (size_t)L.chunk * L.MP * 2);
    L.rec = off; off = al(off + (size_t)L.super * sizeof(Rec));
    L.trec = off; off = al(off + (size_t)L.chunk * (L.HWp / CN) * sizeof(TileRec));
    L.wpk = off; off = al(off + 256 * 4);
    L.kstar = off; off = al(off + (size_t)L.super * 4);
    L.xwin = off; off = al(off + (size_t)L.super * WX * WX * 4);
    L.HWk = (g->ph + 7) / 8 * 8 * g->pw;
    L.nkeys = g->T * L.HWk;
    L.nblocks = (L.nkeys + SCAN_PER_BLOCK - 1) / SCAN_PER_BLOCK;
    L.snorm = off; off = al(off + (size_t)L.super * 4);
    L.rown = off; off = al(off + (size_t)L.super * 4);
    L.perm = off; off = al(off + (size_t)L.super * 4);
    L.hist = off; off = al(off + (size_t)L.nkeys * 4);
    L.cursor = off; off = al(off + (size_t)L.nkeys * 4);
    L.off = off; off = al(off + (size_t)(L.nkeys + 1) * 4);
    L.bsum = off; off = al(off + (size_t)(L.nblocks + 1) * 4);
    L.nvalid = off; off = al(off + 16);
    L.cap = (M + CM - 1) / CM * CM;
    L.redo_cnt = off; off = al(off + 16);
    L.redo_lists = off; off = al(off + (size_t)3 * L.cap * 4);
    L.unc_lists = off; off = al(off + (size_t)3 * L.cap * 4);
    L.exact = off;
    const int redo_rows = L.super < 65536 ? L.super : 65536;
    L.total = off + (size_t)redo_rows * (((size_t)g->ph * g->pw + 63) / 64 * 64 + 1) * sizeof(float);
    return L;
}

}

size_t dtk_track_mfma_workspace_bytes(const dtk_geom* g, int M, int round_sources) {
    return mfma_layout(g, M, round_sources).total;
}

#ifdef DTK_DEV
extern "C" int dtk_debug_counters(unsigned long long* out4) {
    unsigned long long z[4] = {0, 0, 0, 0};
    DTK_HIP(hipMemcpyFromSymbol(out4, HIP_SYMBOL(g_dbg), sizeof(z)));
    DTK_HIP(hipMemcpyToSymbol(HIP_SYMBOL(g_dbg), z, sizeof(z)));
    return DTK_OK;
}
#endif

extern "C" size_t dtk_feat_f16_bytes(const dtk_geom* g) {
    if (!g || g->T <= 0 || g->C <= 0) return 0;
    const size_t unit = (size_t)g->T * hw_pad(g->ph, g->pw) * g->C * 2;
    (void)unit;
    return rc_scale_offset(g) + 256;
}

extern "C" int dtk_make_feat_f16(const dtk_geom* g, const float* feat, const float* norms, void* feat_f16, void* stream) {
    DTK_REQUIRE(g && feat && norms && feat_f16, "dtk_make_feat_f16: null pointer");
    DTK_REQUIRE(g->C % CK == 0, "dtk_make_feat_f16: C=%d must be a multiple of %d for the MFMA path", g->C, CK);
    const int HWp = hw_pad(g->ph, g->pw);
    const long long cells = (long long)g->T * HWp;
    DTK_LAUNCH("feat16", feat16_kernel, dim3(dtk_cdiv(cells, 4)), dim3(256), 0, dtk_stream(stream), feat, norms,
               reinterpret_cast<half_t*>(feat_f16), g->T, g->ph, g->pw, pw_pad(g->pw), g->C);
    unsigned* slot = reinterpret_cast<unsigned*>(reinterpret_cast<unsigned char*>(feat_f16) + rc_scale_offset(g));
    DTK_HIP(dtk_zero_async(slot, 256, dtk_stream(stream)));
    {
        const long long nn = (long long)g->T * g->ph * g->pw;
        const int blocks = (int)(dtk_cdiv(nn, 256) < 512 ? dtk_cdiv(nn, 256) : 512);
        DTK_LAUNCH("rcscale", rcscale_max_kernel, dim3(blocks), dim3(256), 0, dtk_stream(stream), norms, nn, slot);
        DTK_LAUNCH("rcscale", rcscale_final_kernel, dim3(1), dim3(1), 0, dtk_stream(stream), slot);
    }
    if (has_split_planes(g)) {
        const long long n8 = (long long)g->T * g->ph * g->pw * g->C / 8;
        DTK_LAUNCH("featsplit", featsplit_kernel, dim3(dtk_cdiv(n8, 256)), dim3(256), 0, dtk_stream(stream), feat,
                   reinterpret_cast<half_t*>(reinterpret_cast<unsigned char*>(feat_f16) + split_planes_offset(g)), n8,
                   reinterpret_cast<const float*>(slot));
    }
    return DTK_OK;
}

namespace {

struct SrcLists {
    const int32_t *src_row, *tgt, *out_idx;
};

int mfma_phase(const dtk_geom* g, const MfmaLayout& L, unsigned char* ws, const float* feat, const float* norms,
               const half_t* f16, const float* head, const float* emb, SrcLists in, float* out_xy, int count,
               int normalized, bool fast, Redo redo, Redo uncert, size_t lds_head, hipStream_t st, int dbg,
               int32_t* arg_cell = nullptr, float* arg_cos = nullptr, bool row_table = false) {
    half_t* s16 = reinterpret_cast<half_t*>(ws + L.s16);
    half_t* maps = reinterpret_cast<half_t*>(ws + L.maps);
    Rec* rec = reinterpret_cast<Rec*>(ws + L.rec);
    uint32_t* wpk = reinterpret_cast<uint32_t*>(ws + L.wpk);
    int32_t* kstar = reinterpret_cast<int32_t*>(ws + L.kstar);
    float* xwin = reinterpret_cast<float*>(ws + L.xwin);
    int32_t* hist = reinterpret_cast<int32_t*>(ws + L.hist);
    int32_t* cursor = reinterpret_cast<int32_t*>(ws + L.cursor);
    int32_t* koff = reinterpret_cast<int32_t*>(ws + L.off);
    int32_t* bsum = reinterpret_cast<int32_t*>(ws + L.bsum);
    int32_t* nvalid = reinterpret_cast<int32_t*>(ws + L.nvalid);
    float* snorm = reinterpret_cast<float*>(ws + L.snorm);
    int32_t* perm = reinterpret_cast<int32_t*>(ws + L.perm);
    const int32_t* nodm = nullptr;
    const int M = count;
    for (long long s0 = 0; s0 < M; s0 += L.super) {
        const int scnt = (int)((M - s0) < L.super ? (M - s0) : L.super);
        const int pk_cb = DTK_DBG(dbg, 65536) ? 2 : PK_CB, pk_cells = 32 * pk_cb;
        const bool peaks_shape = L.HWp / pk_cells <= (1 << (PK_IDX_BITS - (pk_cb > 1 ? 5 : 4))) &&
                                 L.HWp % pk_cells == 0 && pw_pad(g->pw) % pk_cells == 0 && !DTK_DBG(dbg, 2048) &&
                                 (long long)g->T * L.HWp * g->C * 2 < (1LL << 32);
        const bool peaks_wide = fast && peaks_wide_ok(g->C) && pk_cb == 1 && peaks_shape;
        const bool peaks = (fast && g->C == 384 && peaks_shape) || peaks_wide;
        DTK_HIP(hipMemsetAsync(ws + L.hist, 0, L.cursor + (size_t)L.nkeys * 4 - L.hist, st));
        if (peaks) {
            const int32_t* row_of = row_table ? in.src_row : nullptr;
            if (!row_of)
                DTK_LAUNCH("src16", src16_kernel, dim3(dtk_cdiv(scnt, 4)), dim3(256), 0, st, emb, in.src_row, s16, (int)s0, scnt, M,
                           nodm, g->C, PK_SRC_SCALE, (float*)nullptr);
            const dim3 pgrid(dtk_cdiv(scnt, peaks_wide ? PKW_SRC : PK_SRC));
            const bool fuse_done = row_table && arg_cell == nullptr && !DTK_DBG(dbg, 2);
            const PeaksDone pdone = fuse_done ? PeaksDone{kstar, snorm, hist, reinterpret_cast<const float*>(ws + L.rown), L.HWk}
                                              : PeaksDone{nullptr, nullptr, nullptr, nullptr, 0};
#define DTK_PEAKS(V, CBV)                                                                                                    \
    do {                                                                                                                     \
        static const hipError_t attr_ = hipFuncSetAttribute(reinterpret_cast<const void*>(&corr_peaks_kernel<24, V, CBV>),  \
                                                            hipFuncAttributeMaxDynamicSharedMemorySize,                      \
                                                            (int)peaks_lds_bytes(CBV));                                      \
        DTK_HIP(attr_);                                                                                                      \
        DTK_LAUNCH("corr_peaks", (corr_peaks_kernel<24, V, CBV>), pgrid, dim3(256), peaks_lds_bytes(CBV), st, *g, f16, s16,  \
                   in.tgt, rec, (int)s0, scnt, L.HWp, row_of, pdone);                                                        \
    } while (0)
#define DTK_PEAKS_WIDE(KSHV)                                                                                                  \
    do {                                                                                                                     \
        static const hipError_t attr_ = hipFuncSetAttribute(reinterpret_cast<const void*>(&corr_peaks_wide_kernel<KSHV>),   \
                                                            hipFuncAttributeMaxDynamicSharedMemorySize,                      \
                                                            (int)peaks_wide_lds_bytes(32 * KSHV));                           \
        DTK_HIP(attr_);                                                                                                      \
        DTK_LAUNCH("corr_peaks", (corr_peaks_wide_kernel<KSHV>), pgrid, dim3(256), peaks_wide_lds_bytes(32 * KSHV), st, *g,  \
                   f16, s16, in.tgt, rec, (int)s0, scnt, L.HWp, row_of, pdone);                                              \
    } while (0)
            if (peaks_wide) {
                if (g->C == 1024) DTK_PEAKS_WIDE(32);
                else DTK_PEAKS_WIDE(24);
            } else
#ifdef DTK_DEV
            if (pk_cb == 2) {
                switch ((dbg >> 13) & 7) {
                    case 0: DTK_PEAKS(0, 2); break;
                    case 1: DTK_PEAKS(1, 2); break;
                    case 2: DTK_PEAKS(2, 2); break;
                    case 4: DTK_PEAKS(4, 2); break;
                    default: DTK_PEAKS(7, 2); break;
                }
            } else {
                switch ((dbg >> 13) & 7) {
                    case 0: DTK_PEAKS(0, PK_CB); break;
                    case 1: DTK_PEAKS(1, PK_CB); break;
                    case 2: DTK_PEAKS(2, PK_CB); break;
// ... 184 lines not shown
```

### dino_tracker_amd/csrc/vit.hip

```cpp
#include <stdlib.h>
#include "common.h"
#include "vit_attention4.h"
#include "vit_attention6.h"
#include "vit_gemm_common.h"
#include "vit_gemm_tiled.h"
#include "vit_gemm_ws.h"
#include "vit_gemm_ws_ln.h"
#include "vit_gemm_wide.h"
#include "vit_split.h"

namespace {

__global__ __launch_bounds__(256) void patch_embed_kernel(const float* __restrict__ frames, const float* __restrict__ Wp,
                                                          const float* __restrict__ bp, const float* __restrict__ pos,
                                                          const float* __restrict__ cls_pos,
                                                          const float* __restrict__ mean_std, float* __restrict__ x,
                                                          int H, int W, int ph, int pw, int D, int patch, int stride,
                                                          int S) {
    const int HW = ph * pw;
    const int K = 3 * patch * patch;
    const int frame = blockIdx.z;
    const int tid = threadIdx.x, lane = tid & 63, w = tid >> 6;
    const int p0 = blockIdx.x * 64 + (w >> 1) * 32;
    const int n0 = blockIdx.y * 64 + (w & 1) * 32;
// ... 114 lines not shown
#pragma unroll
            for (int n = 0; n < 3; ++n) {
                const int wo = (n * 32 + li) * PE_WP + ls * 16 + hh * 8;
                const h8 wh = *reinterpret_cast<const h8*>(Wsh + wo), wl = *reinterpret_cast<const h8*>(Wsl + wo);
                acc[n] = __builtin_amdgcn_mfma_f32_32x32x16_f16(xl, wh, acc[n], 0, 0, 0);
                acc[n] = __builtin_amdgcn_mfma_f32_32x32x16_f16(xh, wl, acc[n], 0, 0, 0);
                acc[n] = __builtin_amdgcn_mfma_f32_32x32x16_f16(xh, wh, acc[n], 0, 0, 0);
            }
        }
    }
#pragma unroll
    for (int n = 0; n < 3; ++n) {
        const int co = n0 + n * 32 + li;
        if (co >= D) continue;
        const float b = bp[co];
#pragma unroll
        for (int r = 0; r < 16; ++r) {
            const int pc = pc0 + w * 32 + (r & 3) + 8 * (r >> 2) + 4 * hh;
            if (pc < pw) {
                const int pp = pr * pw + pc;
                x[((size_t)frame * S + 1 + pp) * D + co] = acc[n][r] * (1.f / PE_WSCALE) + b + pos[(size_t)pp * D + co];
            }
        }
        if (pr == 0 && pc0 == 0 && w == 0 && hh == 0) x[(size_t)frame * S * D + co] = cls_pos[co];
    }
}

template <typename T, int NIT = 4>
__global__ __launch_bounds__(256) void layernorm_kernel(float* __restrict__ x, const T* __restrict__ delta,
                                                        const float* __restrict__ gam, const float* __restrict__ bet,
                                                        T* __restrict__ y, long long rows, int D, float eps,
                                                        int* __restrict__ overflow) {
    typedef typename Vec<T>::t8 T8;
    typedef typename Vec<T>::t4 T4;
    (void)sizeof(T8); (void)sizeof(T4);
    operand_mode<T>();
    const long long row = (long long)blockIdx.x * 4 + (threadIdx.x >> 6);
    if (row >= rows) return;
    const int lane = threadIdx.x & 63;
    float* p = x + row * D;
    float4 v[NIT];
    float s = 0.f;
    bool sat = false;
#pragma unroll
    for (int it = 0; it < NIT; ++it) {
        const int c = lane * 4 + it * 256;
        if (c < D) {
            v[it] = *reinterpret_cast<const float4*>(p + c);
            if (delta) {
                const T4 d = *reinterpret_cast<const T4*>(delta + row * D + c);
                const float d0 = (float)d[0], d1 = (float)d[1], d2 = (float)d[2], d3 = (float)d[3];
                if (IsF16<T>::value) sat |= !(fmaxf(fmaxf(fabsf(d0), fabsf(d1)), fmaxf(fabsf(d2), fabsf(d3))) < 65504.f);
                v[it].x += d0; v[it].y += d1; v[it].z += d2; v[it].w += d3;
                *reinterpret_cast<float4*>(p + c) = v[it];
            }
            s += (v[it].x + v[it].y) + (v[it].z + v[it].w);
        }
    }
    if (IsF16<T>::value && overflow && __any(sat) && lane == 0) atomicOr(overflow, 1);
    const float mean = wave_sum(s) / (float)D;
    float q = 0.f;
#pragma unroll
    for (int it = 0; it < NIT; ++it) {
        if (lane * 4 + it * 256 < D) {
            const float a = v[it].x - mean, b = v[it].y - mean, cc = v[it].z - mean, d = v[it].w - mean;
            q += (a * a + b * b) + (cc * cc + d * d);
        }
    }
    const float rstd = rsqrtf(wave_sum(q) / (float)D + eps);
    if (!y) return;
    T* o = y + row * D;
#pragma unroll
    for (int it = 0; it < NIT; ++it) {
        const int c = lane * 4 + it * 256;
        if (c < D) {
            const float4 g = *reinterpret_cast<const float4*>(gam + c), b = *reinterpret_cast<const float4*>(bet + c);
            T4 r = {(T)((v[it].x - mean) * rstd * g.x + b.x), (T)((v[it].y - mean) * rstd * g.y + b.y),
                     (T)((v[it].z - mean) * rstd * g.z + b.z), (T)((v[it].w - mean) * rstd * g.w + b.w)};
            *reinterpret_cast<T4*>(o + c) = r;
        }
    }
}

__global__ __launch_bounds__(256) void zero_kernel(uint4* __restrict__ p, long long n16) {
    const long long i = (long long)blockIdx.x * 256 + threadIdx.x;
    if (i < n16) p[i] = make_uint4(0, 0, 0, 0);
}

template <typename T>
__global__ __launch_bounds__(256) void final_update_kernel(const float* __restrict__ x, const T* __restrict__ delta,
                                                           float* __restrict__ tokens_out, float* __restrict__ feat_out, int S, int D,
                                                           long long total4, int* __restrict__ overflow) {
    typedef typename Vec<T>::t4 T4;
    const long long i = (long long)blockIdx.x * 256 + threadIdx.x;
    bool sat = false;
    if (i < total4) {
        const int d4 = D / 4;
        const long long row = i / d4;
        const int c = (int)(i - row * d4);
        const long long f = row / S, s = row - f * S;
        float4 v = reinterpret_cast<const float4*>(x)[i];
        const T4 d = reinterpret_cast<const T4*>(delta)[i];
        const float d0 = (float)d[0], d1 = (float)d[1], d2 = (float)d[2], d3 = (float)d[3];
        if (IsF16<T>::value) sat = !(fmaxf(fmaxf(fabsf(d0), fabsf(d1)), fmaxf(fabsf(d2), fabsf(d3))) < 65504.f);
        v.x += d0; v.y += d1; v.z += d2; v.w += d3;
        if (tokens_out) reinterpret_cast<float4*>(tokens_out)[i] = v;
        if (feat_out && s > 0) reinterpret_cast<float4*>(feat_out)[(f * (S - 1) + s - 1) * d4 + c] = v;
    }
    if (IsF16<T>::value && overflow && __any(sat) && (threadIdx.x & 63) == 0) atomicOr(overflow, 1);
}

template <typename T>
__global__ __launch_bounds__(256) void tap_kernel(const float* __restrict__ x, const T* __restrict__ delta, float* __restrict__ out,
                                                  float scale, long long total4) {
    typedef typename Vec<T>::t4 T4;
    const long long i = (long long)blockIdx.x * 256 + threadIdx.x;
    if (i >= total4) return;
    float4 v = reinterpret_cast<const float4*>(x)[i];
    if (delta) {
        const T4 d = reinterpret_cast<const T4*>(delta)[i];
        v.x += (float)d[0]; v.y += (float)d[1]; v.z += (float)d[2]; v.w += (float)d[3];
    }
    float4 o = reinterpret_cast<float4*>(out)[i];
    o.x += scale * v.x; o.y += scale * v.y; o.z += scale * v.z; o.w += scale * v.w;
    reinterpret_cast<float4*>(out)[i] = o;
}

__global__ __launch_bounds__(256) void drop_cls_kernel(const float* __restrict__ x, float* __restrict__ out, int S, int D,
                                                       long long total4) {
    const long long i = (long long)blockIdx.x * 256 + threadIdx.x;
    if (i >= total4) return;
    const int d4 = D / 4;
    const long long row = i / d4;
    const int c = (int)(i - row * d4);
    const long long f = row / (S - 1), s = row - f * (S - 1);
    reinterpret_cast<float4*>(out)[i] = reinterpret_cast<const float4*>(x)[(f * S + 1 + s) * d4 + c];
}

constexpr int VIT_FRAME_BATCH = 90;

struct VitPlan {
    int S, Sp, FB;
    size_t x, xn, q, k, vt, ao, hid, delta, total;
    bool split;
    size_t xn_lo, q_lo, k_lo, vt_lo, ao_lo, hid_lo;
};

inline bool vit_layer_split(const dtk_vit_layer& L) { return L.qkv_w_lo != nullptr; }

VitPlan vit_plan(const dtk_vit_model* m, int ph, int pw, int frames) {
    VitPlan p;
    p.S = ph * pw + 1;
    p.Sp = (p.S + 127) / 128 * 128;
    const int fb = m->frame_batch > 0 ? m->frame_batch : VIT_FRAME_BATCH;
    p.FB = frames < fb ? frames : fb;
    auto al = [](size_t v) { return (v + 255) & ~(size_t)255; };
    size_t off = 0;
    const size_t rows = (size_t)p.FB * p.S;
    p.x = off; off = al(off + rows * m->D * 4);
    p.xn = off; off = al(off + rows * m->D * 2);
    p.q = off; off = al(off + (size_t)p.FB * m->heads * p.Sp * 64 * 2);
    p.k = off; off = al(off + (size_t)p.FB * m->heads * p.Sp * 64 * 2);
    p.vt = off; off = al(off + (size_t)p.FB * m->heads * p.Sp * 64 * 2);
    p.ao = off; off = al(off + rows * m->D * 2);
    p.hid = off; off = al(off + rows * 4 * m->D * 2);
    p.delta = off; off = al(off + rows * m->D * 2);
    p.split = false;
    for (int l = 0; l < m->depth; ++l) p.split |= vit_layer_split(m->layers[l]);
    p.xn_lo = p.q_lo = p.k_lo = p.vt_lo = p.ao_lo = p.hid_lo = 0;
// ... 87 lines not shown
                return DTK_OK;
            }
        }
        if (path.ws && K == WS_K && ws_fits) {
            const auto gr = gemm_ws_grid(N, rows);
            if (path.ws_v1)
                DTK_LAUNCH(name, (gemm_ws_kernel<T, EPI, 0>), gr.first, dim3(256), 0, st, A, W, rows, N, e, gr.second);
            else if (N % 64 != 0 || DTK_DBG(e.no_store, 128))
                DTK_LAUNCH(name, (gemm_ws_kernel<T, EPI, 3, false>), gr.first, dim3(256), 0, st, A, W, rows, N, e, gr.second);
            else
                DTK_LAUNCH(name, (gemm_ws_kernel<T, EPI>), gr.first, dim3(256), 0, st, A, W, rows, N, e, gr.second);
            return DTK_OK;
        }
        if (path.ws && EPI == EPI_DELTA) {
            const dim3 grid(dtk_cdiv(rows, WD_M));
            if (path.wide_v1)
                DTK_LAUNCH(name, (gemm_wide_delta_kernel<T, false>), grid, dim3(512), 0, st, A, W, rows, K, e);
            else if (e.ln_out)
                DTK_LAUNCH(name, (gemm_wide_delta_kernel<T, true, true>), grid, dim3(512), 0, st, A, W, rows, K, e);
            else
                DTK_LAUNCH(name, (gemm_wide_delta_kernel<T, true>), grid, dim3(512), 0, st, A, W, rows, K, e);
            return DTK_OK;
        }
        if (path.wide) {
            const dim3 grid(gemm_wide_grid(N, rows));
            if (path.wide_v1)
                DTK_LAUNCH(name, (gemm_wide_kernel<T, EPI, false>), grid, dim3(512), 0, st, A, W, rows, N, K, e);
            else
                DTK_LAUNCH(name, (gemm_wide_kernel<T, EPI, true>), grid, dim3(512), 0, st, A, W, rows, N, K, e);
            return DTK_OK;
        }
    }
    DTK_LAUNCH(name, (gemm_tiled_kernel<T, EPI>), dim3(gemm_grid(N, rows)), dim3(256), 0, st, A, W, rows, N, K, e);
    return DTK_OK;
}

template <typename T>
int launch_gemm_swiglu(const char* name, const GemmPath& path, const T* A, const T* W, long long rows, int N, int K, const GemmEpi<T>& e,
                       hipStream_t st) {
    if (path.wide)
        DTK_LAUNCH(name, (gemm_wide_kernel<T, EPI_SWIGLU, true>), dim3(gemm_wide_grid(N, rows)), dim3(512), 0, st, A, W, rows, N, K, e);
    else
        DTK_LAUNCH(name, (gemm_tiled_kernel<T, EPI_SWIGLU>), dim3(gemm_grid(N, rows)), dim3(256), 0, st, A, W, rows, N, K, e);
    return DTK_OK;
}
inline bool vit_swiglu_flags_ok(int flags, const char* who) {
    if (!(flags & (DTK_VIT_GEMM_WIDE_V1 | DTK_VIT_GEMM_WS_V1))) return true;
    dtk_set_error("%s: the SwiGLU feed-forward has no A / B kernel forms: clear %s", who,
                  (flags & DTK_VIT_GEMM_WIDE_V1) ? "DTK_VIT_GEMM_WIDE_V1" : "DTK_VIT_GEMM_WS_V1");
    return false;
}

template <typename T, int SEPI>
int launch_gemm_split(const char* name, const GemmPath& path, const T* Ah, const T* Al, const T* Wh, const T* Wl, long long rows,
                      int N, int K, const SplitEpi<T>& se, hipStream_t st) {
    if (!path.tiled && N % SD_N == 0) {
        const dim3 grid(gemm_split_dma_grid(N, rows));
        if constexpr (SEPI == SEPI_SWIGLU)
            DTK_LAUNCH(name, (gemm_split_dma_kernel<T, SEPI, true>), grid, dim3(512), 0, st, Ah, Al, Wh, Wl, rows, N, K, se);
        else if (path.wide_v1)
            DTK_LAUNCH(name, (gemm_split_dma_kernel<T, SEPI, false>), grid, dim3(512), 0, st, Ah, Al, Wh, Wl, rows, N, K, se);
        else
            DTK_LAUNCH(name, (gemm_split_dma_kernel<T, SEPI, true>), grid, dim3(512), 0, st, Ah, Al, Wh, Wl, rows, N, K, se);
        return DTK_OK;
    }
    DTK_LAUNCH(name, (gemm_split_kernel<T, SEPI>), dim3(gemm_split_grid(N, rows)), dim3(256), 0, st, Ah, Al, Wh, Wl, rows, N, K, se);
    return DTK_OK;
}

template <typename T>
int vit_run(const dtk_vit_model* m, const float* frames, int nframes, int video_h, int video_w, float* tokens_out,
            float* feat_out, float* qkv_out, unsigned char* ws, const VitPlan& p, int ph, int pw, hipStream_t st) {
    const int HW = ph * pw, D = m->D;
    const bool swiglu = m->ffn == DTK_VIT_FFN_SWIGLU;
    const int HID = m->hidden > 0 ? m->hidden : 4 * D;
    float* x = reinterpret_cast<float*>(ws + p.x);
    auto at = [&](size_t off) { return reinterpret_cast<T*>(ws + off); };
    T *xn = at(p.xn), *q = at(p.q), *k = at(p.k), *vt = at(p.vt), *ao = at(p.ao), *hid = at(p.hid), *delta = at(p.delta);
    T *xn_lo = at(p.xn_lo), *q_lo = at(p.q_lo), *k_lo = at(p.k_lo), *vt_lo = at(p.vt_lo), *ao_lo = at(p.ao_lo), *hid_lo = at(p.hid_lo);
    int* ovf = m->overflow;
    const bool scan_all = ovf && (m->flags & DTK_VIT_CHECK_RANGE);
    int* const epi_ovf = IsF16<T>::value ? ovf : nullptr;
    const int S = p.S, Sp = p.Sp;
    {
        const long long n16 = (long long)((p.ao - p.q) / 16);
        DTK_LAUNCH("vit_zero", zero_kernel, dim3(dtk_cdiv(n16, 256)), dim3(256), 0, st, reinterpret_cast<uint4*>(q), n16);
        if (p.split) {
            const long long m16 = (long long)((p.ao_lo - p.q_lo) / 16);
            DTK_LAUNCH("vit_zero", zero_kernel, dim3(dtk_cdiv(m16, 256)), dim3(256), 0, st, reinterpret_cast<uint4*>(q_lo), m16);
        }
    }
    for (int f0 = 0; f0 < nframes; f0 += p.FB) {
        const int nf = (nframes - f0) < p.FB ? (nframes - f0) : p.FB;
        const long long rows = (long long)nf * S;
        auto scan_range = [&](const T* t, long long n, int bit) -> int {
            const int blocks = (int)(dtk_cdiv(n / 8, 256) < 1024 ? dtk_cdiv(n / 8, 256) : 1024);
            DTK_LAUNCH("vit_range_scan", range_scan_kernel<T>, dim3(blocks), dim3(256), 0, st, t, n / 8, ovf, bit);
            return DTK_OK;
        };
        const bool pe_fits = (size_t)nf * video_h * video_w * 16 <= p.delta - p.hid &&
                             (size_t)D * PE_K * 4 <= p.total - p.delta;
        if (m->patch == PE_P && m->stride == PE_S && pe_fits) {
            h4v* fh = reinterpret_cast<h4v*>(hid);
            h4v* fl = fh + (size_t)nf * video_h * video_w;
            half_t* wh = reinterpret_cast<half_t*>(delta);
            half_t* wl = wh + (size_t)D * PE_K;
            const long long npix = (long long)nf * video_h * video_w;
            DTK_LAUNCH("vit_frame_split", frame_split4_kernel, dim3(dtk_cdiv(npix, 256)), dim3(256), 0, st,
                       frames + (size_t)f0 * 3 * video_h * video_w, m->mean_std, fh, fl, video_h, video_w, npix);
            DTK_LAUNCH("vit_frame_split", pack_patch_split_kernel, dim3(dtk_cdiv((long long)D * PE_K, 256)), dim3(256), 0, st,
                       m->patch_w, D, wh, wl);
            const int groups_x = dtk_cdiv(pw, PE_TOK);
            const int units = groups_x * ph * nf, slabs = dtk_cdiv(D, PE_NF);
            DTK_LAUNCH("vit_patch_embed", patch_embed_split_kernel, dim3(8 * dtk_cdiv(units, 8) * slabs), dim3(256), 0, st, fh,
                       fl, wh, wl, m->patch_b, m->pos, m->cls_pos, x, video_h, video_w, ph, pw, D, S, groups_x, units, slabs);
        } else {
            DTK_LAUNCH("vit_patch_embed", patch_embed_kernel, dim3(dtk_cdiv(HW, 64), dtk_cdiv(D, 64), nf), dim3(256), 0, st,
                       frames + (size_t)f0 * 3 * video_h * video_w, m->patch_w, m->patch_b, m->pos, m->cls_pos, m->mean_std,
                       x, video_h, video_w, ph, pw, D, m->patch, m->stride, S);
        }
        const GemmPath path = gemm_path(m);
        const int dbg_ns = DTK_DBG(dtk_dev_flags() >> 16, 0xff);
        bool pending = false;
        bool ln1_done = false;
        auto tap = [&](int l, bool with_delta) -> int {
            if (!m->tap_out || !((m->tap_mask >> l) & 1)) return DTK_OK;
            const long long t4 = rows * (D / 4);
            DTK_LAUNCH("vit_tap", tap_kernel<T>, dim3(dtk_cdiv(t4, 256)), dim3(256), 0, st, x, with_delta ? (const T*)delta : (const T*)nullptr,
                       m->tap_out + (size_t)f0 * S * D, m->tap_scale, t4);
            return DTK_OK;
        };
        for (int l = 0; l < m->depth; ++l) {
            const dtk_vit_layer& L = m->layers[l];
            const T* qkv_w = reinterpret_cast<const T*>(L.qkv_w);
            const T* proj_w = reinterpret_cast<const T*>(L.proj_w);
            const T* fc1_w = reinterpret_cast<const T*>(L.fc1_w);
            const T* fc2_w = reinterpret_cast<const T*>(L.fc2_w);
            if (vit_layer_split(L)) {
                const T* qkv_wl = reinterpret_cast<const T*>(L.qkv_w_lo);
                const T* proj_wl = reinterpret_cast<const T*>(L.proj_w_lo);
                const T* fc1_wl = reinterpret_cast<const T*>(L.fc1_w_lo);
                const T* fc2_wl = reinterpret_cast<const T*>(L.fc2_w_lo);
                const float inv_ws = 1.f / (L.w_scale > 0.f ? L.w_scale : 1.f);
                if (launch_layernorm_split<T>(x, pending ? (const T*)delta : (const T*)nullptr, L.ln1_w, L.ln1_b, xn, xn_lo, rows, D, m->ln_eps,
                                              ovf, st)) return DTK_E_HIP;
                pending = false;
                SplitEpi<T> se{};
                if (qkv_out && l == m->depth - 1) {
                    se.bias = L.qkv_b; se.inv_wscale = inv_ws; se.out_f32 = qkv_out + (size_t)f0 * S * 3 * D;
                    if (launch_gemm_split<T, SEPI_F32>("vit_gemm_qkv_facet", path, xn, xn_lo, qkv_w, qkv_wl, rows, 3 * D, D, se, st)) return DTK_E_HIP;
                    se = SplitEpi<T>{};
                }
                se.bias = L.qkv_b; se.inv_wscale = inv_ws; se.q_hi = q; se.q_lo = q_lo; se.k_hi = k; se.k_lo = k_lo; se.vt_hi = vt;
                se.vt_lo = vt_lo; se.S = S; se.Sp = Sp; se.heads = m->heads; se.D = D; se.qscale = 0.125f * 1.4426950408889634f;
                se.ovf = epi_ovf;
                if (launch_gemm_split<T, SEPI_QKV>("vit_gemm_qkv_split", path, xn, xn_lo, qkv_w, qkv_wl, rows, 3 * D, D, se, st)) return DTK_E_HIP;
                const int nqb = dtk_cdiv(Sp, 128);
                DTK_LAUNCH("vit_attention_split", attention_split_kernel<T>, dim3((unsigned)(nf * m->heads * nqb)), dim3(256), 0, st,
                           (const T*)q, (const T*)q_lo, (const T*)k, (const T*)k_lo, (const T*)vt, (const T*)vt_lo, ao, ao_lo, S, Sp,
                           m->heads, nqb);
                se = SplitEpi<T>{};
                se.bias = L.proj_b; se.inv_wscale = inv_ws; se.x = x; se.gamma = L.ls1;
                if (launch_gemm_split<T, SEPI_RESID>("vit_gemm_proj_split", path, ao, ao_lo, proj_w, proj_wl, rows, D, D, se, st)) return DTK_E_HIP;
                if (launch_layernorm_split<T>(x, (const T*)nullptr, L.ln2_w, L.ln2_b, xn, xn_lo, rows, D, m->ln_eps, ovf, st)) return DTK_E_HIP;
                se = SplitEpi<T>{};
                se.bias = L.fc1_b; se.inv_wscale = inv_ws; se.out_hi = hid; se.out_lo = hid_lo; se.ovf = epi_ovf;
                if (swiglu ? launch_gemm_split<T, SEPI_SWIGLU>("vit_gemm_fc1_split", path, xn, xn_lo, fc1_w, fc1_wl, rows, 2 * HID, D, se, st)
                           : launch_gemm_split<T, SEPI_GELU>("vit_gemm_fc1_split", path, xn, xn_lo, fc1_w, fc1_wl, rows, HID, D, se, st)) return DTK_E_HIP;
                se = SplitEpi<T>{};
                se.bias = L.fc2_b; se.inv_wscale = inv_ws; se.x = x; se.gamma = L.ls2;
                if (launch_gemm_split<T, SEPI_RESID>("vit_gemm_fc2_split", path, hid, hid_lo, fc2_w, fc2_wl, rows, D, HID, se, st)) return DTK_E_HIP;
                if (tap(l, false)) return DTK_E_HIP;
                continue;
// ... 266 lines not shown
```

### dino_tracker_amd/ops.py

```python
from __future__ import annotations

from typing import Dict, Optional, Tuple

import torch

from . import _lib
from ._lib import Geom, TrackOpts, TrackStats, check, lib

TRACK_EXACT, TRACK_MFMA = 0, 1
TIER_AUTO, TIER_WHOLE_MAP = 0, 1


def _p(t: Optional[torch.Tensor], dtype: Optional[torch.dtype] = None):
    if t is None:
        return None
    if not t.is_cuda:
        raise RuntimeError("dino_tracker_amd: tensor is not on a GPU -- the hot path has no CPU fallback")
    if not t.is_contiguous():
        raise RuntimeError("dino_tracker_amd: tensor must be contiguous")
    if dtype is not None and t.dtype != dtype:
        raise RuntimeError(f"dino_tracker_amd: expected {dtype}, got {t.dtype}")
    return t.data_ptr()


# ... 263 lines not shown
    cov = torch.empty((C, C), dtype=torch.float32, device=x.device)
    nb = int(lib().dtk_pca_moments_workspace_bytes(N, C, int(chunk_rows)))
    ws = torch.empty(max(nb, 1), dtype=torch.uint8, device=x.device)
    check(lib().dtk_pca_moments(_p(x, torch.float32), N, C, int(bool(normalize)), int(chunk_rows), _p(mean), _p(cov), _p(ws), nb,
                                _stream()))
    return mean, cov


def pca_project(x: torch.Tensor, V: torch.Tensor, normalize: bool = True) -> Tuple[torch.Tensor, torch.Tensor]:
    N, C = _pca_rows(x)
    if V.dim() != 2 or V.shape[1] != C or not 1 <= V.shape[0] <= PCA_MAX_Q:
        raise RuntimeError(f"dino_tracker_amd: V must be [q <= {PCA_MAX_Q}, {C}], got {tuple(V.shape)}")
    q = int(V.shape[0])
    colors = torch.empty((N, q), dtype=torch.float32, device=x.device)
    minmax = torch.empty(2 * PCA_MAX_Q, dtype=torch.float32, device=x.device)
    nb = int(lib().dtk_pca_project_workspace_bytes(N))
    ws = torch.empty(nb, dtype=torch.uint8, device=x.device)
    check(lib().dtk_pca_project(_p(x, torch.float32), N, C, int(bool(normalize)), _p(V, torch.float32), q, _p(colors), _p(minmax),
                                _p(ws), nb, _stream()))
    return colors, minmax


def fg_mask(colors: torch.Tensor, minmax: torch.Tensor, grid: Tuple[int, int, int], img_size: Tuple[int, int], threshold: float,
            comp: int = 0, flip: bool = False) -> Tuple[torch.Tensor, torch.Tensor]:
    T, h, w = (int(v) for v in grid)
    H, W = (int(v) for v in img_size)
    if colors.dim() != 2 or colors.shape[0] != T * h * w or minmax.shape != (2 * PCA_MAX_Q,):
        raise RuntimeError(f"dino_tracker_amd: fg_mask: colors {tuple(colors.shape)} / minmax {tuple(minmax.shape)} do not fit "
                           f"the grid {T}x{h}x{w}")
    mask = torch.empty((T, H, W), dtype=torch.uint8, device=colors.device)
    tok = torch.empty((T, h, w), dtype=torch.uint8, device=colors.device)
    check(lib().dtk_fg_mask(_p(colors, torch.float32), int(colors.shape[1]), int(comp), _p(minmax, torch.float32), float(threshold),
                            int(bool(flip)), T, h, w, H, W, _p(mask), _p(tok), _stream()))
    return mask, tok


def traj_cos_sims(S: torch.Tensor, tq: torch.Tensor, N: int, T: int) -> torch.Tensor:
    C = S.shape[-1]
    cs = torch.empty((N, T), dtype=torch.float32, device=S.device)
    check(lib().dtk_traj_cos_sims(_p(S, torch.float32), _p(tq, torch.int32), _p(cs), N, T, C, _stream()))
    return cs


class AnchorSources:

    def __init__(self, N: int, T: int, device):
        i32 = dict(dtype=torch.int32, device=device)
        self.N, self.T = N, T
        self.n_anchors = torch.empty(N, **i32)
        self.pair_off = torch.empty(N + 1, **i32)
        self.pair_frame = torch.empty(N * T, **i32)
        self.src_row = torch.empty(N * T * T, **i32)
        self.tgt = torch.empty(N * T * T, **i32)
        self.out_idx = torch.empty(N * T * T, **i32)
        self.counts = torch.zeros(4, **i32)
        self.scratch = torch.empty(2 * T + 2 + N, **i32)


def build_anchor_sources(cs: torch.Tensor, anchor_th: float, buf: Optional[AnchorSources] = None) -> AnchorSources:
    N, T = cs.shape
    if buf is None or buf.N != N or buf.T != T:
        buf = AnchorSources(N, T, cs.device)
    check(lib().dtk_build_anchor_sources(_p(cs, torch.float32), float(anchor_th), N, T, _p(buf.n_anchors),
                                         _p(buf.pair_off), _p(buf.pair_frame), _p(buf.src_row), _p(buf.tgt),
                                         _p(buf.out_idx), _p(buf.counts), _p(buf.scratch), _stream()))
    return buf


def build_anchor_sources_needed(cs: torch.Tensor, anchor_th: float, cos_th: float,
                                buf: Optional[AnchorSources] = None) -> AnchorSources:
    N, T = cs.shape
    if buf is None or buf.N != N or buf.T != T:
        buf = AnchorSources(N, T, cs.device)
    check(lib().dtk_build_anchor_sources_needed(_p(cs, torch.float32), float(anchor_th), float(cos_th), N, T,
                                                _p(buf.n_anchors), _p(buf.pair_off), _p(buf.pair_frame), _p(buf.src_row),
                                                _p(buf.tgt), _p(buf.out_idx), _p(buf.counts), _p(buf.scratch), _stream()))
    return buf


def occlusion(green: torch.Tensor, pair_off: torch.Tensor, pair_frame: torch.Tensor, traj: torch.Tensor,
              cs: torch.Tensor, anchor_th: float, cos_th: float, needed_only: bool = False) -> torch.Tensor:
    N, T = cs.shape
    occ = torch.empty((N, T), dtype=torch.uint8, device=cs.device)
    fn = lib().dtk_occlusion_needed if needed_only else lib().dtk_occlusion
    check(fn(_p(green, torch.float32), _p(pair_off, torch.int32), _p(pair_frame, torch.int32), _p(traj, torch.float32),
             _p(cs, torch.float32), float(anchor_th), float(cos_th), _p(occ), N, T, _stream()))
    return occ.bool()


def profile_enable(on: bool) -> None:
    check(lib().dtk_profile_enable(int(on)))


def profile_collect() -> Dict[str, Tuple[float, int]]:
    n = lib().dtk_profile_collect()
    return {lib().dtk_profile_name(i).decode(): (lib().dtk_profile_ms(i), lib().dtk_profile_launches(i)) for i in range(n)}


def batchnorm_train_forward(x: torch.Tensor, gamma: torch.Tensor, beta: torch.Tensor, running_mean: Optional[torch.Tensor],
                            running_var: Optional[torch.Tensor], momentum: float, eps: float, relu: bool,
                            pre_bias: Optional[torch.Tensor] = None):
    N, C, H, W = x.shape
    y = torch.empty_like(x)
    mean = torch.empty(C, dtype=torch.float32, device=x.device)
    rstd = torch.empty(C, dtype=torch.float32, device=x.device)
    nb = int(lib().dtk_batchnorm_workspace_bytes(C))
    ws = torch.empty(nb, dtype=torch.uint8, device=x.device)
    check(lib().dtk_batchnorm_train_forward(_p(x, torch.float32), _p(gamma, torch.float32), _p(beta, torch.float32),
                                            _p(pre_bias, torch.float32), _p(running_mean, torch.float32),
                                            _p(running_var, torch.float32), float(momentum),
                                            float(eps), int(relu), _p(y), _p(mean), _p(rstd), N, C, H * W, _p(ws), nb, _stream()))
    for buf in (running_mean, running_var):
        if buf is not None:
            torch.autograd.graph.increment_version(buf)
    return y, mean, rstd


def batchnorm_train_backward(x: torch.Tensor, dy: torch.Tensor, gamma: torch.Tensor, beta: torch.Tensor, mean: torch.Tensor,
                             rstd: torch.Tensor, relu: bool, want_pre_bias: bool = False):
    N, C, H, W = x.shape
    dx = torch.empty_like(x)
    dgamma = torch.empty(C, dtype=torch.float32, device=x.device)
    dbeta = torch.empty(C, dtype=torch.float32, device=x.device)
    dpre = torch.empty(C, dtype=torch.float32, device=x.device) if want_pre_bias else None
    nb = int(lib().dtk_batchnorm_workspace_bytes(C))
    ws = torch.empty(nb, dtype=torch.uint8, device=x.device)
    check(lib().dtk_batchnorm_train_backward(_p(x, torch.float32), _p(dy, torch.float32), _p(gamma, torch.float32),
                                             _p(beta, torch.float32), _p(mean, torch.float32), _p(rstd, torch.float32),
                                             int(relu), _p(dx), _p(dgamma), _p(dbeta), _p(dpre), N, C, H * W, _p(ws), nb,
                                             _stream()))
    return dx, dgamma, dbeta, dpre


def blurpool_forward(x: torch.Tensor) -> torch.Tensor:
    N, C, H, W = x.shape
    y = torch.empty((N, C, (H - 1) // 2 + 1, (W - 1) // 2 + 1), dtype=torch.float32, device=x.device)
    check(lib().dtk_blurpool_forward(_p(x, torch.float32), _p(y), N * C, H, W, _stream()))
    return y


def blurpool_backward(dy: torch.Tensor, H: int, W: int) -> torch.Tensor:
    N, C, Ho, Wo = dy.shape
    if (Ho, Wo) != ((H - 1) // 2 + 1, (W - 1) // 2 + 1):
        raise RuntimeError(f"blurpool_backward: {Ho}x{Wo} is not the pooled size of {H}x{W}")
    dx = torch.empty((N, C, H, W), dtype=torch.float32, device=dy.device)
    check(lib().dtk_blurpool_backward(_p(dy, torch.float32), _p(dx), N * C, H, W, _stream()))
    return dx


def gemm_nt(A: torch.Tensor, B: torch.Tensor, C: torch.Tensor, M: int, N: int, K: int, lda: int, ldb: int, ldc: int,
            batch: int = 1, stride_a: int = 0, stride_b: int = 0, stride_c: int = 0, split_k: int = 1, accumulate: int = 0,
            scale_a: Optional[torch.Tensor] = None, scale_b: Optional[torch.Tensor] = None) -> None:
    check(lib().dtk_gemm_nt_f32(_p(A, torch.float32), _p(B, torch.float32), _p(C, torch.float32), M, N, K, lda, ldb, ldc, batch,
                                stride_a, stride_b, stride_c, split_k, accumulate, _p(scale_a, torch.float32),
                                _p(scale_b, torch.float32), _stream()))


def im2col(x: torch.Tensor, cols: torch.Tensor, ksize: int, pad: int, dil: int, reflect: bool, layout: int, Kp: int,
           Lp: int = 0) -> None:
    n, C, H, W = x.shape
    check(lib().dtk_im2col(_p(x, torch.float32), _p(cols, torch.float32), n, C, H, W, ksize, pad, dil, int(reflect), layout, Kp, Lp,
                           _stream()))


def col2im(dcols: torch.Tensor, dx: torch.Tensor, ksize: int, pad: int, dil: int, reflect: bool, Kp: int) -> None:
    n, C, H, W = dx.shape
    check(lib().dtk_col2im(_p(dcols, torch.float32), _p(dx, torch.float32), n, C, H, W, ksize, pad, dil, int(reflect), Kp, _stream()))


# ... 290 lines not shown
```

### include/dtk.h

```cpp
#ifndef DTK_H_
#define DTK_H_

#include <stddef.h>
#include <stdint.h>

#ifdef __cplusplus
extern "C" {
#endif

#define DTK_OK 0
#define DTK_E_INVALID (-1)
#define DTK_E_HIP (-2)
#define DTK_E_WORKSPACE (-3)

typedef struct dtk_geom {
    int32_t T;
    int32_t C;
    int32_t ph, pw;
    int32_t video_h, video_w;
    int32_t patch, stride;
    float radius;
} dtk_geom;

#define DTK_HEAD_HIDDEN 16
// ... 139 lines not shown
size_t dtk_conv_wgrad_split_workspace_bytes(int N, int Cin, int Cout, int H, int W, int dilation);
int dtk_conv_wgrad_split(const float* x, const float* dy, float* dw, int N, int Cin, int Cout, int H, int W, int dilation,
                         int reflect_pad, const float* scale_dy, int fp16_only, void* workspace, size_t workspace_bytes,
                         void* stream);

size_t dtk_contrastive_workspace_bytes(int Q, int B, int C, int n);
int dtk_contrastive_forward(const float* fe, const float* a, const int32_t* fidx, float temp, int Q, int B, int C, int n, int F,
                            float* fet, float* nf, float* na, float* S, float* lse, void* stream);
int dtk_contrastive_backward(const float* fe, const float* a, const int32_t* fidx, float temp, int Q, int B, int C, int n, int F,
                             const float* nf, const float* na, const float* S, const float* lse, const float* g, float* da,
                             float* dfe, void* workspace, size_t workspace_bytes, void* stream);

int dtk_emb_reg_forward(const float* x, const float* raw, int F, int C, int n, float* cell_sums, float* out2, void* stream);
int dtk_emb_reg_backward(const float* x, const float* raw, const float* cell_sums, const float* grad_out2, int F, int C, int n,
                         float* dx, void* stream);

int dtk_corr_window_backward(const dtk_geom* g, const float* feat, const float* norms, const float* emb, const int32_t* tgt,
                             const float* maps, const float* dmaps, const float* stats, float* demb, float* dfeat, int B,
                             void* stream);

int dtk_normalized_conv2d(const float* x, const float* w, const float* bias, float* y, int B, int Cin, int Cout, int H,
                          int W, int k, void* stream);

int dtk_corr_maps(const dtk_geom* g, const float* feat, const float* norms, const float* emb, const int32_t* src_row,
                  const int32_t* tgt, float* maps, float* snorm_scratch, int M, int relu, void* stream);

#define DTK_TRACK_EXACT 0
#define DTK_TRACK_MFMA 1
#define DTK_TIER_AUTO 0
#define DTK_TIER_WHOLE_MAP 1
typedef struct dtk_track_opts {
    int32_t method, normalized, round_sources, tier;
    int32_t emb_rows;
} dtk_track_opts;
typedef struct dtk_track_stats {
    int32_t sources;
    int32_t whole_map_tier;
    int32_t exact_tier;
    int32_t syncs;
} dtk_track_stats;
size_t dtk_track_workspace_bytes(const dtk_geom* g, int M, const dtk_track_opts* opts);
int dtk_track(const dtk_geom* g, const float* feat, const float* norms, const void* feat_f16,
              const float* head, const float* emb, const int32_t* src_row, const int32_t* tgt,
              const int32_t* out_idx, float* out_xy, int M, const int32_t* dM, const dtk_track_opts* opts,
              dtk_track_stats* stats, void* workspace, size_t workspace_bytes, void* stream);

int dtk_argmax_cells(const dtk_geom* g, const float* feat, const float* norms, const void* feat_f16, const float* emb,
                     const int32_t* src_row, const int32_t* tgt, int32_t* arg_cell, float* arg_cos, int M, int method,
                     void* workspace, size_t workspace_bytes, void* stream);

size_t dtk_bb_nms_workspace_bytes(const dtk_geom* g, int M);
int dtk_bb_nms(const dtk_geom* g, const float* feat, const float* norms, const float* emb, const int32_t* src_row,
               const int32_t* tgt, float box_size, float iou_thresh, int topk, float* peak_affs, float* r, int M,
               void* workspace, size_t workspace_bytes, void* stream);

int dtk_traj_start_fg(const float* traj, int N, int T, const uint8_t* masks, int Tm, int H, int W, uint8_t* fg, int32_t* err,
                      void* stream);

size_t dtk_nearest_traj_workspace_bytes(int N, int T, int gh, int gw);
int dtk_nearest_traj(const float* traj, int N, int T, int gh, int gw, float origin, float stride, int32_t* idx,
                     void* workspace, size_t workspace_bytes, void* stream);

int dtk_of_filter_keep(const float* traj, int N, int T, const int32_t* idx, int gh, int gw, float origin, float stride,
                       const float* src, const float* tgt, const int32_t* pair_off, const int32_t* pair_st, int P,
                       uint8_t* keep, int32_t* err, void* stream);

size_t dtk_feat_f16_bytes(const dtk_geom* g);
int dtk_make_feat_f16(const dtk_geom* g, const float* feat, const float* norms, void* feat_f16, void* stream);

int dtk_traj_cos_sims(const float* S, const int32_t* tq, float* cs, int N, int T, int C, void* stream);

int dtk_build_anchor_sources(const float* cs, float anchor_th, int N, int T, int32_t* n_anchors, int32_t* pair_off,
                             int32_t* pair_frame, int32_t* src_row, int32_t* tgt, int32_t* out_idx,
                             int32_t* counts, int32_t* scratch, void* stream);

int dtk_build_anchor_sources_needed(const float* cs, float anchor_th, float cos_th, int N, int T, int32_t* n_anchors,
                                    int32_t* pair_off, int32_t* pair_frame, int32_t* src_row, int32_t* tgt, int32_t* out_idx,
                                    int32_t* counts, int32_t* scratch, void* stream);

int dtk_occlusion(const float* green, const int32_t* pair_off, const int32_t* pair_frame, const float* traj,
                  const float* cs, float anchor_th, float cos_th, uint8_t* occ, int N, int T, void* stream);

int dtk_occlusion_needed(const float* green, const int32_t* pair_off, const int32_t* pair_frame, const float* traj,
                         const float* cs, float anchor_th, float cos_th, uint8_t* occ, int N, int T, void* stream);

int dtk_tapvid_counts(const float* pred_tracks, const uint8_t* pred_occluded, const float* gt_tracks,
                      const uint8_t* gt_occluded, const int32_t* query_frame, float pred_scale_x, float pred_scale_y,
                      float gt_scale_x, float gt_scale_y, int first_mode, int N, int T, unsigned long long* counts18,
                      void* stream);

int dtk_badja_counts(const float* pred_tracks, const double* gt_tracks, const uint8_t* gt_occluded, const void* segmentations,
                     int32_t seg_is_float, float pred_scale_x, float pred_scale_y, int32_t N, int32_t T, int32_t T_seg,
                     int32_t H, int32_t W, unsigned long long* areas, unsigned long long* counts3, void* stream);

size_t dtk_batchnorm_workspace_bytes(int32_t C);
int dtk_batchnorm_train_forward(const float* x, const float* gamma, const float* beta, const float* pre_bias,
                                float* running_mean, float* running_var, float momentum, float eps, int32_t relu, float* y,
                                float* save_mean, float* save_rstd, int32_t N, int32_t C, int32_t HW, void* workspace,
                                size_t workspace_bytes, void* stream);
int dtk_batchnorm_train_backward(const float* x, const float* dy, const float* gamma, const float* beta,
                                 const float* save_mean, const float* save_rstd, int32_t relu, float* dx, float* dgamma,
                                 float* dbeta, float* dpre_bias, int32_t N, int32_t C, int32_t HW, void* workspace,
                                 size_t workspace_bytes, void* stream);

int dtk_blurpool_forward(const float* x, float* y, int64_t planes, int32_t H, int32_t W, void* stream);
int dtk_blurpool_backward(const float* dy, float* dx, int64_t planes, int32_t H, int32_t W, void* stream);

int dtk_gemm_nt_f32(const float* A, const float* B, float* C, int32_t M, int32_t N, int32_t K, int64_t lda, int64_t ldb,
                    int64_t ldc, int32_t batch, int64_t stride_a, int64_t stride_b, int64_t stride_c, int32_t split_k,
                    int32_t accumulate, const float* scale_a, const float* scale_b, void* stream);
int dtk_gemm_nt_f32_indexed(const float* A, const float* B, float* C, int32_t M, int32_t N, int32_t K, int64_t lda, int64_t ldb,
                            int64_t ldc, int32_t batch, int64_t stride_a, int64_t stride_b, int64_t stride_c, int32_t split_k,
                            int32_t accumulate, const float* scale_a, const float* scale_b, const int32_t* index_b,
                            const int32_t* index_c, void* stream);
int dtk_im2col(const float* x, float* cols, int32_t n, int32_t C, int32_t H, int32_t W, int32_t ksize, int32_t pad, int32_t dil,
               int32_t reflect, int32_t layout, int32_t Kp, int64_t Lp, void* stream);
int dtk_col2im(const float* dcols, float* dx, int32_t n, int32_t C, int32_t H, int32_t W, int32_t ksize, int32_t pad, int32_t dil,
               int32_t reflect, int32_t Kp, void* stream);
int dtk_transpose_f32(const float* src, float* dst, int64_t rows, int64_t cols, int32_t batch, void* stream);

int dtk_resample2d_forward(const float* src, float* dst, int64_t planes, int32_t hs, int32_t ws, int32_t hd, int32_t wd,
                           const int32_t* ylo, const float* ywhi, const int32_t* xlo, const float* xwhi, void* stream);
int dtk_resample2d_backward(const float* ddst, float* dsrc, int64_t planes, int32_t hs, int32_t ws, int32_t hd, int32_t wd,
                            const int32_t* yranges, const float* ywhi, const int32_t* xranges, const float* xwhi, void* stream);

int dtk_sample_bilinear_forward(const float* feat, const float* pts, float* out, int32_t B, int32_t n, int32_t h, int32_t w, int32_t C,
                                void* stream);
int dtk_sample_bilinear_backward(const float* g, const float* pts, float* dfeat, int32_t B, int32_t n, int32_t h, int32_t w, int32_t C,
                                 void* stream);

int dtk_pow2_scale(const float* x, int64_t n, float* out, void* scratch, void* stream);

#define DTK_ADAM_MAX_TENSORS 32
#define DTK_ADAM_MAX_GROUPS 4
typedef struct dtk_adam_args {
    float* param[DTK_ADAM_MAX_TENSORS];
    const float* grad[DTK_ADAM_MAX_TENSORS];
    float* exp_avg[DTK_ADAM_MAX_TENSORS];
    float* exp_avg_sq[DTK_ADAM_MAX_TENSORS];
    int64_t numel[DTK_ADAM_MAX_TENSORS];
    int32_t group[DTK_ADAM_MAX_TENSORS];
    int32_t step[DTK_ADAM_MAX_TENSORS];
    int32_t n_tensors;
    double lr[DTK_ADAM_MAX_GROUPS];
    double beta1, beta2, eps;
} dtk_adam_args;
int dtk_adam_step(const dtk_adam_args* a, void* stream);
int dtk_adam_scalars(const dtk_adam_args* a, float* out_host);
int dtk_adam_step_dev(const dtk_adam_args* a, const float* scalars_dev, void* stream);

size_t dtk_pca_moments_workspace_bytes(int64_t N, int32_t C, int64_t chunk_rows);
int dtk_pca_moments(const float* x, int64_t N, int32_t C, int32_t normalize, int64_t chunk_rows, float* mean, float* cov,
                    void* workspace, size_t workspace_bytes, void* stream);
size_t dtk_pca_project_workspace_bytes(int64_t N);
int dtk_pca_project(const float* x, int64_t N, int32_t C, int32_t normalize, const float* V, int32_t q, float* colors,
                    float* minmax, void* workspace, size_t workspace_bytes, void* stream);
int dtk_fg_mask(const float* colors, int32_t q, int32_t comp, const float* minmax, float thr, int32_t flip, int32_t T, int32_t h,
                int32_t w, int32_t H, int32_t W, uint8_t* mask, uint8_t* token_mask, void* stream);

int dtk_flow_pack(const float* flow, float* packed, int32_t n, int32_t h, int32_t w, void* stream);
int dtk_flow_cycle_masks(const float* fflow_packed, const float* bflow_packed, int32_t T, int32_t h, int32_t w, float threshold,
                         uint8_t* consistent, void* stream);
size_t dtk_flow_traj_workspace_bytes(int32_t T, int32_t h, int32_t w);
int dtk_flow_traj_start(const float* fflow_packed, const float* bflow_packed, const uint8_t* consistent, const uint8_t* visited,
                        int32_t T, int32_t h, int32_t w, int32_t s, float threshold, int32_t min_trajectory_length,
                        const float* direct_fwd, const float* direct_back, int32_t use_direct, float direct_threshold,
                        int32_t* n_rows, void* workspace, size_t workspace_bytes, void* stream);
// ... 97 lines not shown
```

Baseline: 527,500 query-points*frames/s.

## Split occlusion medians across frame groups, add sparse correlation path, fuse feature splitting

The pruned occlusion path becomes two kernels: one computes per-frame anchor-distance medians in parallel over a 2D grid of queries and frame groups, writing them to a scratch buffer, and a second derives the threshold and flags. The exact correlation kernel gains a sparse variant that handles tiles with few live rows, using double-buffered shared memory and register prefetch. The hi/lo fp16 split of features is fused into the feat16 conversion kernel, and the ViT zero-fill now clears only the padded rows instead of whole buffers. Together these aim to raise parallelism in occlusion and cut wasted work and extra memory passes, at the cost of more launches, a scratch allocation and more code complexity.

```diff
diff --git a/dino_tracker_amd/_lib.py b/dino_tracker_amd/_lib.py
--- a/dino_tracker_amd/_lib.py
+++ b/dino_tracker_amd/_lib.py
@@ -187,8 +187,8 @@
                               c_int, c_void_p]),
     "dtk_build_anchor_sources_needed": (c_int, [c_void_p, c_float, c_float, c_int, c_int, c_void_p, c_void_p, c_void_p,
                                                 c_void_p, c_void_p, c_void_p, c_void_p, c_void_p, c_void_p]),
-    "dtk_occlusion_needed": (c_int, [c_void_p, c_void_p, c_void_p, c_void_p, c_void_p, c_float, c_float, c_void_p, c_int,
-                                     c_int, c_void_p]),
+    "dtk_occlusion_needed": (c_int, [c_void_p, c_void_p, c_void_p, c_void_p, c_void_p, c_float, c_float, c_void_p, c_void_p,
+                                     c_int, c_int, c_void_p]),
     "dtk_tapvid_counts": (c_int, [c_void_p, c_void_p, c_void_p, c_void_p, c_void_p, c_float, c_float, c_float, c_float,
                                   c_int, c_int, c_int, c_void_p, c_void_p]),
     "dtk_badja_counts": (c_int, [c_void_p, c_void_p, c_void_p, c_void_p, c_int, c_float, c_float, c_int, c_int, c_int, c_int, c_int,
diff --git a/dino_tracker_amd/csrc/anchors.hip b/dino_tracker_amd/csrc/anchors.hip
--- a/dino_tracker_amd/csrc/anchors.hip
+++ b/dino_tracker_amd/csrc/anchors.hip
@@ -195,7 +195,6 @@
     return sqrtf(__fadd_rn(__fmul_rn(dx, dx), __fmul_rn(dy, dy)));
 }
 
-template <bool PRUNED>
 __global__ __launch_bounds__(256) void occlusion_kernel(const float* __restrict__ green,
                                                         const int32_t* __restrict__ pair_off,
                                                         const int32_t* __restrict__ pair_frame,
@@ -214,18 +213,8 @@
         for (int t = threadIdx.x; t < T; t += 256) occ[(size_t)n * T + t] = 1;
         return;
     }
-    if constexpr (PRUNED) {
-        int undecided = 0;
-        for (int t = threadIdx.x; t < T; t += 256) undecided |= is_undecided(cs[(size_t)n * T + t], anchor_th, cos_th) ? 1 : 0;
-        if (!__syncthreads_or(undecided)) {
-            for (int t = threadIdx.x; t < T; t += 256) occ[(size_t)n * T + t] = cs[(size_t)n * T + t] < cos_th ? 1 : 0;
-            return;
-        }
-    }
     const int want = (A - 1) / 2;
     for (int t = w; t < T; t += 4) {
-        if constexpr (PRUNED)
-            if (!is_needed(cs[(size_t)n * T + t], anchor_th, cos_th)) continue;
         for (int k = lane; k < A; k += WAVE) d[k] = anchor_dist(green, tr, p0 + k, pair_frame[p0 + k], T, t);
         __builtin_amdgcn_fence(__ATOMIC_RELEASE, "wavefront");
         __builtin_amdgcn_wave_barrier();
@@ -251,7 +240,73 @@
     tau = fmaxf(fmaxf(red[0], red[1]), fmaxf(red[2], red[3]));
     for (int t = threadIdx.x; t < T; t += 256) {
         const float c = cs[(size_t)n * T + t];
-        const bool far = (!PRUNED || is_needed(c, anchor_th, cos_th)) && med[t] > tau;
+        const bool far = med[t] > tau;
+        occ[(size_t)n * T + t] = (far || c < cos_th) ? 1 : 0;
+    }
+}
+
+__global__ __launch_bounds__(256) void occlusion_medians_kernel(const float* __restrict__ green, const int32_t* __restrict__ pair_off,
+                                                                const int32_t* __restrict__ pair_frame,
+                                                                const float* __restrict__ traj, const float* __restrict__ cs,
+                                                                float anchor_th, float cos_th, float* __restrict__ med, int N, int T) {
+    extern __shared__ float smem_occ[];
+    const int n = blockIdx.x;
+    const int lane = threadIdx.x & 63, w = threadIdx.x >> 6;
+    float* d = smem_occ + w * T;
+    const int p0 = pair_off[n], A = pair_off[n + 1] - p0;
+    if (A <= 0) return;
+    int undecided = 0;
+    for (int t = threadIdx.x; t < T; t += 256) undecided |= is_undecided(cs[(size_t)n * T + t], anchor_th, cos_th) ? 1 : 0;
+    if (!__syncthreads_or(undecided)) return;
+    const float* tr = traj + (size_t)n * T * 2;
+    const int want = (A - 1) / 2;
+    for (int t = blockIdx.y * 4 + w; t < T; t += 4 * gridDim.y) {
+        if (!is_needed(cs[(size_t)n * T + t], anchor_th, cos_th)) continue;
+        for (int k = lane; k < A; k += WAVE) d[k] = anchor_dist(green, tr, p0 + k, pair_frame[p0 + k], T, t);
+        __builtin_amdgcn_fence(__ATOMIC_RELEASE, "wavefront");
+        __builtin_amdgcn_wave_barrier();
+        for (int k = lane; k < A; k += WAVE) {
+            const float dk = d[k];
+            int rank = 0;
+            for (int k2 = 0; k2 < A; ++k2) {
+                const float d2 = d[k2];
+                rank += (d2 < dk || (d2 == dk && k2 < k)) ? 1 : 0;
+            }
+            if (rank == want) med[(size_t)n * T + t] = dk;
+        }
+        __builtin_amdgcn_fence(__ATOMIC_RELEASE, "wavefront");
+        __builtin_amdgcn_wave_barrier();
+    }
+}
+
+__global__ __launch_bounds__(256) void occlusion_flags_kernel(const int32_t* __restrict__ pair_off, const float* __restrict__ cs,
+                                                              float anchor_th, float cos_th, const float* __restrict__ med,
+                                                              uint8_t* __restrict__ occ, int N, int T) {
+    __shared__ float red[4];
+    const int n = blockIdx.x;
+    const int lane = threadIdx.x & 63, w = threadIdx.x >> 6;
+    const float* c_ = cs + (size_t)n * T;
+    const float* m_ = med + (size_t)n * T;
+    if (pair_off[n + 1] - pair_off[n] <= 0) {
+        for (int t = threadIdx.x; t < T; t += 256) occ[(size_t)n * T + t] = 1;
+        return;
+    }
+    int undecided = 0;
+    for (int t = threadIdx.x; t < T; t += 256) undecided |= is_undecided(c_[t], anchor_th, cos_th) ? 1 : 0;
+    if (!__syncthreads_or(undecided)) {
+        for (int t = threadIdx.x; t < T; t += 256) occ[(size_t)n * T + t] = c_[t] < cos_th ? 1 : 0;
+        return;
+    }
+    float tau = -INFINITY;
+    for (int t = threadIdx.x; t < T; t += 256)
+        if (c_[t] >= anchor_th) tau = fmaxf(tau, m_[t]);
+    tau = wave_max(tau);
+    if (lane == 0) red[w] = tau;
+    __syncthreads();
+    tau = fmaxf(fmaxf(red[0], red[1]), fmaxf(red[2], red[3]));
+    for (int t = threadIdx.x; t < T; t += 256) {
+        const float c = c_[t];
+        const bool far = is_needed(c, anchor_th, cos_th) && m_[t] > tau;
         occ[(size_t)n * T + t] = (far || c < cos_th) ? 1 : 0;
     }
 }
@@ -282,7 +337,7 @@
     DTK_REQUIRE(green && pair_off && pair_frame && traj && cs && occ && N >= 0 && T > 0, "dtk_occlusion: bad args");
     DTK_REQUIRE((size_t)5 * T * sizeof(float) <= 60 * 1024, "dtk_occlusion: T=%d too large", T);
     if (N == 0) return DTK_OK;
-    DTK_LAUNCH("occlusion", occlusion_kernel<false>, dim3(N), dim3(256), (size_t)5 * T * sizeof(float), dtk_stream(stream), green,
+    DTK_LAUNCH("occlusion", occlusion_kernel, dim3(N), dim3(256), (size_t)5 * T * sizeof(float), dtk_stream(stream), green,
                        pair_off, pair_frame, traj, cs, anchor_th, cos_th, occ, N, T);
     return DTK_OK;
 }
@@ -310,12 +365,16 @@
 }
 
 extern "C" int dtk_occlusion_needed(const float* green, const int32_t* pair_off, const int32_t* pair_frame, const float* traj,
-                                    const float* cs, float anchor_th, float cos_th, uint8_t* occ, int N, int T, void* stream) {
-    DTK_REQUIRE(green && pair_off && pair_frame && traj && cs && occ && N >= 0 && T > 0, "dtk_occlusion_needed: bad args");
+                                    const float* cs, float anchor_th, float cos_th, uint8_t* occ, float* med_scratch, int N, int T,
+                                    void* stream) {
+    DTK_REQUIRE(green && pair_off && pair_frame && traj && cs && occ && med_scratch && N >= 0 && T > 0, "dtk_occlusion_needed: bad args");
     DTK_REQUIRE((size_t)5 * T * sizeof(float) <= 60 * 1024, "dtk_occlusion_needed: T=%d too large", T);
     if (N == 0) return DTK_OK;
-    DTK_LAUNCH("occlusion", occlusion_kernel<true>, dim3(N), dim3(256), (size_t)5 * T * sizeof(float), dtk_stream(stream), green,
-                       pair_off, pair_frame, traj, cs, anchor_th, cos_th, occ, N, T);
+    const int groups = dtk_cdiv(T, 8) < 64 ? dtk_cdiv(T, 8) : 64;
+    DTK_LAUNCH("occlusion_medians", occlusion_medians_kernel, dim3(N, groups), dim3(256), (size_t)4 * T * sizeof(float),
+               dtk_stream(stream), green, pair_off, pair_frame, traj, cs, anchor_th, cos_th, med_scratch, N, T);
+    DTK_LAUNCH("occlusion", occlusion_flags_kernel, dim3(N), dim3(256), 0, dtk_stream(stream), pair_off, cs, anchor_th, cos_th,
+               (const float*)med_scratch, occ, N, T);
     return DTK_OK;
 }
 
diff --git a/dino_tracker_amd/csrc/track_exact.hip b/dino_tracker_amd/csrc/track_exact.hip
--- a/dino_tracker_amd/csrc/track_exact.hip
+++ b/dino_tracker_amd/csrc/track_exact.hip
@@ -5,6 +5,13 @@
 namespace {
 
 constexpr int TM = 64, TN = 64, TK = 16;
+constexpr int PF = 8;
+constexpr int SPARSE_ROWS = 8;
+
+__device__ __forceinline__ int nth_set_bit(unsigned long long m, int n) {
+    for (int i = 0; i < n; ++i) m &= m - 1;
+    return __ffsll((long long)m) - 1;
+}
 constexpr int HR = 6;
 constexpr int HR_LARGE = 2;
 
@@ -52,6 +59,7 @@
     if (lane == 0) snorm[i] = sqrtf(s);
 }
 
+template <bool SPARSE>
 __global__ __launch_bounds__(256) void corr_exact_kernel(dtk_geom g, const float* __restrict__ feat,
                                                          const float* __restrict__ norms,
                                                          const float* __restrict__ emb,
@@ -60,8 +68,8 @@
                                                          const float* __restrict__ snorm, float* __restrict__ maps,
                                                          int m0, int count, int M, const int32_t* __restrict__ dM,
                                                          int HWs, int relu) {
-    __shared__ __attribute__((aligned(16))) float As[TK][TM + 4];
-    __shared__ __attribute__((aligned(16))) float Bs[TK][TN + 4];
+    __shared__ __attribute__((aligned(16))) float As[2][TK][TM + 4];
+    __shared__ __attribute__((aligned(16))) float Bs[2][TK][TN + 4];
     __shared__ int s_tgt[TM];
     __shared__ int s_row[TM];
     __shared__ int s_fr[2];
@@ -91,54 +99,126 @@
     }
     __syncthreads();
     const int fmin = s_fr[0], fmax = s_fr[1];
-    const int ty = tid >> 4, tx = tid & 15;
+    const int ty = tid >> 4, tx = tid & 15, lane = tid & 63, wv = tid >> 6;
     const int lr = tid >> 2, lk = (tid & 3) * 4;
     const float* arow = emb + (size_t)s_row[lr] * g.C;
     const int lcell = cell0 + lr;
     for (int f = fmin; f <= fmax; ++f) {
-        bool mine = false;
-#pragma unroll
-        for (int i = 0; i < 4; ++i) mine |= (s_tgt[ty * 4 + i] == f);
-        if (!__syncthreads_or(mine)) continue;
+        const unsigned long long live = __ballot(s_tgt[lane] == f);
+        if (!live) continue;
+        const int nlive = __popcll(live);
         const float* brow = feat + ((size_t)f * HW + min(lcell, HW - 1)) * g.C;
-        float acc[4][4];
-#pragma unroll
-        for (int i = 0; i < 4; ++i)
-#pragma unroll
-            for (int j = 0; j < 4; ++j) acc[i][j] = 0.f;
-        for (int k0 = 0; k0 < g.C; k0 += TK) {
-            float4 a = make_float4(0.f, 0.f, 0.f, 0.f), b = a;
-            if (k0 + lk < g.C) {
-                a = *reinterpret_cast<const float4*>(arow + k0 + lk);
-                if (lcell < HW) b = *reinterpret_cast<const float4*>(brow + k0 + lk);
-            }
-            As[lk + 0][lr] = a.x; As[lk + 1][lr] = a.y; As[lk + 2][lr] = a.z; As[lk + 3][lr] = a.w;
-            Bs[lk + 0][lr] = b.x; Bs[lk + 1][lr] = b.y; Bs[lk + 2][lr] = b.z; Bs[lk + 3][lr] = b.w;
+        if ((nlive <= SPARSE_ROWS) != SPARSE) continue;
+        if constexpr (!SPARSE) {
+            float acc[4][4];
+#pragma unroll
+            for (int i = 0; i < 4; ++i)
+#pragma unroll
+                for (int j = 0; j < 4; ++j) acc[i][j] = 0.f;
+            for (int k0 = 0; k0 < g.C; k0 += TK) {
+                float4 a = make_float4(0.f, 0.f, 0.f, 0.f), b = a;
+                if (k0 + lk < g.C) {
+                    a = *reinterpret_cast<const float4*>(arow + k0 + lk);
+                    if (lcell < HW) b = *reinterpret_cast<const float4*>(brow + k0 + lk);
+                }
+                As[0][lk + 0][lr] = a.x; As[0][lk + 1][lr] = a.y; As[0][lk + 2][lr] = a.z; As[0][lk + 3][lr] = a.w;
+                Bs[0][lk + 0][lr] = b.x; Bs[0][lk + 1][lr] = b.y; Bs[0][lk + 2][lr] = b.z; Bs[0][lk + 3][lr] = b.w;
+                __syncthreads();
+#pragma unroll
+                for (int kk = 0; kk < TK; ++kk) {
+                    const float4 av = *reinterpret_cast<const float4*>(&As[0][kk][ty * 4]);
+                    const float4 bv = *reinterpret_cast<const float4*>(&Bs[0][kk][tx * 4]);
+                    const float aa[4] = {av.x, av.y, av.z, av.w}, bb[4] = {bv.x, bv.y, bv.z, bv.w};
+#pragma unroll
+                    for (int i = 0; i < 4; ++i)
+#pragma unroll
+                        for (int j = 0; j < 4; ++j) acc[i][j] = fmaf(aa[i], bb[j], acc[i][j]);
+                }
+                __syncthreads();
+            }
+#pragma unroll
+            for (int i = 0; i < 4; ++i) {
+                const int r = ty * 4 + i;
+                if (s_tgt[r] != f) continue;
+                const int ml = tile_m0 - m0 + r;
+                const float sn = snorm[ml];
+#pragma unroll
+                for (int j = 0; j < 4; ++j) {
+                    const int cell = cell0 + tx * 4 + j;
+                    if (cell < HW) {
+                        const float den = fmaxf(sn * norms[(size_t)f * HW + cell], 1e-8f);
+                        const float rho = acc[i][j] / den;
+                        maps[(size_t)ml * HWs + cell] = relu ? fmaxf(rho, 0.f) : rho;
+                    }
+                }
+            }
+            continue;
+        }
+        if constexpr (SPARSE) {
+            const bool mine = wv < nlive, two = wv + 4 < nlive;
+            const int r0 = nth_set_bit(live, min(wv, nlive - 1)), r1 = two ? nth_set_bit(live, wv + 4) : r0;
+            float acc2[2] = {0.f, 0.f};
+            const int nsteps = g.C / TK;
+            const bool bkeep = lcell < HW;
+            float4 ra[PF], rb[PF];
+            auto kload = [&](int s, float4& a, float4& b) {
+                a = *reinterpret_cast<const float4*>(arow + s * TK + lk);
+                b = *reinterpret_cast<const float4*>(brow + s * TK + lk);
+            };
+            auto kstore = [&](int st, const float4& a, const float4& b) {
+                As[st][lk + 0][lr] = a.x; As[st][lk + 1][lr] = a.y; As[st][lk + 2][lr] = a.z; As[st][lk + 3][lr] = a.w;
+                Bs[st][lk + 0][lr] = bkeep ? b.x : 0.f; Bs[st][lk + 1][lr] = bkeep ? b.y : 0.f;
+                Bs[st][lk + 2][lr] = bkeep ? b.z : 0.f; Bs[st][lk + 3][lr] = bkeep ? b.w : 0.f;
+            };
+            auto multiply = [&](int st) {
+                if (!mine) return;
+#pragma unroll 4
+                for (int kk = 0; kk < TK; ++kk) {
+                    const float bv = Bs[st][kk][lane];
+                    acc2[0] = fmaf(As[st][kk][r0], bv, acc2[0]);
+                    acc2[1] = fmaf(As[st][kk][r1], bv, acc2[1]);
+                }
+            };
+            if (nsteps >= PF) {
+#pragma unroll
+                for (int u = 0; u < PF; ++u) kload(u, ra[u], rb[u]);
+            } else {
+#pragma unroll
+                for (int u = 0; u < PF; ++u)
+                    if (u < nsteps) kload(u, ra[u], rb[u]);
+            }
+            kstore(0, ra[0], rb[0]);
             __syncthreads();
-#pragma unroll
-            for (int kk = 0; kk < TK; ++kk) {
-                const float4 av = *reinterpret_cast<const float4*>(&As[kk][ty * 4]);
-                const float4 bv = *reinterpret_cast<const float4*>(&Bs[kk][tx * 4]);
-                const float aa[4] = {av.x, av.y, av.z, av.w}, bb[4] = {bv.x, bv.y, bv.z, bv.w};
-#pragma unroll
-                for (int i = 0; i < 4; ++i)
-#pragma unroll
-                    for (int j = 0; j < 4; ++j) acc[i][j] = fmaf(aa[i], bb[j], acc[i][j]);
-            }
-            __syncthreads();
-        }
-#pragma unroll
-        for (int i = 0; i < 4; ++i) {
-            const int r = ty * 4 + i;
-            if (s_tgt[r] != f) continue;
-            const int ml = tile_m0 - m0 + r;
-            const float sn = snorm[ml];
-#pragma unroll
-            for (int j = 0; j < 4; ++j) {
-                const int cell = cell0 + tx * 4 + j;
-                if (cell < HW) {
-                    const float den = fmaxf(sn * norms[(size_t)f * HW + cell], 1e-8f);
-                    const float rho = acc[i][j] / den;
+            int s0 = 0;
+            for (; s0 + 2 * PF <= nsteps; s0 += PF) {
+#pragma unroll
+                for (int u = 0; u < PF; ++u) {
+                    multiply(u & 1);
+                    kstore((u + 1) & 1, ra[(u + 1) % PF], rb[(u + 1) % PF]);
+                    kload(s0 + u + PF, ra[u], rb[u]);
+                    __syncthreads();
+                }
+            }
+            for (; s0 < nsteps; s0 += PF) {
+#pragma unroll
+                for (int u = 0; u < PF; ++u) {
+                    const int s = s0 + u;
+                    if (s >= nsteps) break;
+                    multiply(u & 1);
+                    if (s + 1 < nsteps) kstore((u + 1) & 1, ra[(u + 1) % PF], rb[(u + 1) % PF]);
+                    if (s + PF < nsteps) kload(s + PF, ra[u], rb[u]);
+                    __syncthreads();
+                }
+            }
+            const int cell = cell0 + lane;
+            if (mine && cell < HW) {
+                const float fn = norms[(size_t)f * HW + cell];
+#pragma unroll
+                for (int j = 0; j < 2; ++j) {
+                    if (j && !two) break;
+                    const int ml = tile_m0 - m0 + (j ? r1 : r0);
+                    const float den = fmaxf(snorm[ml] * fn, 1e-8f);
+                    const float rho = acc2[j] / den;
                     maps[(size_t)ml * HWs + cell] = relu ? fmaxf(rho, 0.f) : rho;
                 }
             }
@@ -386,7 +466,9 @@
         const int cnt = (int)((M - m0) < chunk ? (M - m0) : chunk);
         DTK_LAUNCH("row_norms", row_norms_kernel, dim3(dtk_cdiv(cnt, 4)), dim3(256), 0, st, emb, src_row, snorm, (int)m0,
                            cnt, M, dM, g->C);
-        DTK_LAUNCH("corr_exact", corr_exact_kernel, dim3(dtk_cdiv(HW, TN), dtk_cdiv(cnt, TM)), dim3(256), 0, st, *g, feat,
+        DTK_LAUNCH("corr_exact", corr_exact_kernel<false>, dim3(dtk_cdiv(HW, TN), dtk_cdiv(cnt, TM)), dim3(256), 0, st, *g, feat,
+                           norms, emb, src_row, tgt, snorm, maps, (int)m0, cnt, M, dM, HWs, 1);
+        DTK_LAUNCH("corr_exact_sparse", corr_exact_kernel<true>, dim3(dtk_cdiv(HW, TN), dtk_cdiv(cnt, TM)), dim3(256), 0, st, *g, feat,
                            norms, emb, src_row, tgt, snorm, maps, (int)m0, cnt, M, dM, HWs, 1);
         const int rc = launch_head_exact("dtk_track(exact)", "head_exact", g, head, maps, HWs, out_idx, out_xy, (int)m0, cnt, M, dM,
                                          normalized, nullptr, st);
@@ -704,7 +786,10 @@
         const int cnt = (int)((M - m0) < step ? (M - m0) : step);
         DTK_LAUNCH("row_norms", row_norms_kernel, dim3(dtk_cdiv(cnt, 4)), dim3(256), 0, st, emb, src_row, snorm_scratch + m0,
                    (int)m0, cnt, M, (const int32_t*)nullptr, g->C);
-        DTK_LAUNCH("corr_exact", corr_exact_kernel, dim3(dtk_cdiv(HW, TN), dtk_cdiv(cnt, TM)), dim3(256), 0, st, *g, feat,
+        DTK_LAUNCH("corr_exact", corr_exact_kernel<false>, dim3(dtk_cdiv(HW, TN), dtk_cdiv(cnt, TM)), dim3(256), 0, st, *g, feat,
+                   norms, emb, src_row, tgt, snorm_scratch + m0, maps + (size_t)m0 * HW, (int)m0, cnt, M,
+                   (const int32_t*)nullptr, HW, relu);
+        DTK_LAUNCH("corr_exact_sparse", corr_exact_kernel<true>, dim3(dtk_cdiv(HW, TN), dtk_cdiv(cnt, TM)), dim3(256), 0, st, *g, feat,
                    norms, emb, src_row, tgt, snorm_scratch + m0, maps + (size_t)m0 * HW, (int)m0, cnt, M,
                    (const int32_t*)nullptr, HW, relu);
     }
@@ -730,7 +815,9 @@
         const int cnt = (int)((M - m0) < chunk ? (M - m0) : chunk);
         DTK_LAUNCH("row_norms", row_norms_kernel, dim3(dtk_cdiv(cnt, 4)), dim3(256), 0, st, emb, src_row, snorm, (int)m0, cnt, M,
                    (const int32_t*)nullptr, g->C);
-        DTK_LAUNCH("corr_exact", corr_exact_kernel, dim3(dtk_cdiv(HW, TN), dtk_cdiv(cnt, TM)), dim3(256), 0, st, *g, feat, norms,
+        DTK_LAUNCH("corr_exact", corr_exact_kernel<false>, dim3(dtk_cdiv(HW, TN), dtk_cdiv(cnt, TM)), dim3(256), 0, st, *g, feat, norms,
+                   emb, src_row, tgt, snorm, maps, (int)m0, cnt, M, (const int32_t*)nullptr, HWs, 0);
+        DTK_LAUNCH("corr_exact_sparse", corr_exact_kernel<true>, dim3(dtk_cdiv(HW, TN), dtk_cdiv(cnt, TM)), dim3(256), 0, st, *g, feat, norms,
                    emb, src_row, tgt, snorm, maps, (int)m0, cnt, M, (const int32_t*)nullptr, HWs, 0);
         DTK_LAUNCH("argmax_exact", argmax_exact_kernel, dim3(cnt), dim3(256), 0, st, maps, HW, HWs, out_idx, arg_cell, arg_cos,
                    (int)m0, cnt);
@@ -860,7 +947,9 @@
         const int cnt = (int)((M - m0) < chunk ? (M - m0) : chunk);
         DTK_LAUNCH("row_norms", row_norms_kernel, dim3(dtk_cdiv(cnt, 4)), dim3(256), 0, st, emb, src_row, snorm, (int)m0, cnt, M,
                    (const int32_t*)nullptr, g->C);
-        DTK_LAUNCH("corr_exact", corr_exact_kernel, dim3(dtk_cdiv(HW, TN), dtk_cdiv(cnt, TM)), dim3(256), 0, st, *g, feat, norms,
+        DTK_LAUNCH("corr_exact", corr_exact_kernel<false>, dim3(dtk_cdiv(HW, TN), dtk_cdiv(cnt, TM)), dim3(256), 0, st, *g, feat, norms,
+                   emb, src_row, tgt, snorm, maps, (int)m0, cnt, M, (const int32_t*)nullptr, HWs, 0);
+        DTK_LAUNCH("corr_exact_sparse", corr_exact_kernel<true>, dim3(dtk_cdiv(HW, TN), dtk_cdiv(cnt, TM)), dim3(256), 0, st, *g, feat, norms,
                    emb, src_row, tgt, snorm, maps, (int)m0, cnt, M, (const int32_t*)nullptr, HWs, 0);
         DTK_LAUNCH("bb_nms", bb_nms_kernel, dim3(cnt), dim3(256), 0, st, *g, maps, HWs, box_size, iou_thresh, topk, peak_affs, r,
                    (int)m0, cnt);
diff --git a/dino_tracker_amd/csrc/track_mfma.hip b/dino_tracker_amd/csrc/track_mfma.hip
--- a/dino_tracker_amd/csrc/track_mfma.hip
+++ b/dino_tracker_amd/csrc/track_mfma.hip
@@ -38,8 +38,39 @@
 __host__ __device__ inline int map_xw(int pw) { return pw_pad(pw) + 16; }
 __host__ __device__ inline int hw_pad(int ph, int pw) { return ph * pw_pad(pw); }
 
+__host__ __device__ inline bool peaks_wide_ok(int C) { return C == 768 || C == 1024; }
+
+constexpr float RC_SCALE_MAX = 32.f;
+__host__ __device__ inline size_t split_planes_offset(const dtk_geom* g) {
+    return ((size_t)g->T * hw_pad(g->ph, g->pw) * g->C * 2 + 255) / 256 * 256;
+}
+__host__ __device__ inline bool has_split_planes(const dtk_geom* g) {
+    return g->C == 384 && (long long)g->T * g->ph * g->pw * g->C * 4 < (1LL << 32);
+}
+__host__ __device__ inline size_t rc_scale_offset(const dtk_geom* g) {
+    const size_t unit = (size_t)g->T * hw_pad(g->ph, g->pw) * g->C * 2;
+    const size_t end = has_split_planes(g) ? split_planes_offset(g) + (size_t)g->T * g->ph * g->pw * g->C * 4 : unit;
+    return (end + 255) / 256 * 256;
+}
+__global__ __launch_bounds__(256) void rcscale_max_kernel(const float* __restrict__ norms, long long n, unsigned* __restrict__ slot) {
+    float m = 0.f;
+    for (long long i = (long long)blockIdx.x * 256 + threadIdx.x; i < n; i += (long long)gridDim.x * 256) {
+        const float v = norms[i];
+        m = fmaxf(m, v == v ? v : 3.0e38f);
+    }
+    m = wave_max(m);
+    if ((threadIdx.x & 63) == 0) atomicMax(slot + 1, __float_as_uint(m));
+}
+__global__ void rcscale_final_kernel(unsigned* __restrict__ slot) {
+    const float m = __uint_as_float(slot[1]);
+    float sc = RC_SCALE_MAX;
+    while (sc > 0x1p-40f && m * sc > 16384.f) sc *= 0.5f;
+    reinterpret_cast<float*>(slot)[0] = sc;
+}
+template <bool SPLIT>
 __global__ __launch_bounds__(256) void feat16_kernel(const float* __restrict__ feat, const float* __restrict__ norms,
-                                                     half_t* __restrict__ f16, int T, int ph, int pw, int PWP, int C) {
+                                                     half_t* __restrict__ f16, half_t* __restrict__ fs,
+                                                     const float* __restrict__ rc_scale, int T, int ph, int pw, int PWP, int C) {
     const long long cell = (long long)blockIdx.x * 4 + (threadIdx.x >> 6);
     const int HWp = ph * PWP, HW = ph * pw;
     if (cell >= (long long)T * HWp) return;
@@ -51,64 +82,30 @@
         for (int k = lane * 8; k < C; k += 512) *reinterpret_cast<uint4*>(o + k) = make_uint4(0, 0, 0, 0);
         return;
     }
-    const float* p = feat + ((size_t)t * HW + r * pw + c) * C;
-    const float nrm = norms[(size_t)t * HW + r * pw + c];
+    const size_t rc = (size_t)t * HW + r * pw + c;
+    const float* p = feat + rc * C;
+    const float nrm = norms[rc];
     const float sc = nrm > 1e-30f ? FSCALE / nrm : 0.f;
+    const float RC_SCALE = SPLIT ? *rc_scale : 0.f;
     for (int k = lane * 8; k < C; k += 512) {
         const float4 a = *reinterpret_cast<const float4*>(p + k), b = *reinterpret_cast<const float4*>(p + k + 4);
         h8 v = {(half_t)(a.x * sc), (half_t)(a.y * sc), (half_t)(a.z * sc), (half_t)(a.w * sc),
                 (half_t)(b.x * sc), (half_t)(b.y * sc), (half_t)(b.z * sc), (half_t)(b.w * sc)};
         *reinterpret_cast<h8*>(o + k) = v;
-    }
-}
-
-__host__ __device__ inline bool peaks_wide_ok(int C) { return C == 768 || C == 1024; }
-
-constexpr float RC_SCALE_MAX = 32.f;
-__host__ __device__ inline size_t split_planes_offset(const dtk_geom* g) {
-    return ((size_t)g->T * hw_pad(g->ph, g->pw) * g->C * 2 + 255) / 256 * 256;
-}
-__host__ __device__ inline bool has_split_planes(const dtk_geom* g) {
-    return g->C == 384 && (long long)g->T * g->ph * g->pw * g->C * 4 < (1LL << 32);
-}
-__host__ __device__ inline size_t rc_scale_offset(const dtk_geom* g) {
-    const size_t unit = (size_t)g->T * hw_pad(g->ph, g->pw) * g->C * 2;
-    const size_t end = has_split_planes(g) ? split_planes_offset(g) + (size_t)g->T * g->ph * g->pw * g->C * 4 : unit;
-    return (end + 255) / 256 * 256;
-}
-__global__ __launch_bounds__(256) void rcscale_max_kernel(const float* __restrict__ norms, long long n, unsigned* __restrict__ slot) {
-    float m = 0.f;
-    for (long long i = (long long)blockIdx.x * 256 + threadIdx.x; i < n; i += (long long)gridDim.x * 256) {
-        const float v = norms[i];
-        m = fmaxf(m, v == v ? v : 3.0e38f);
-    }
-    m = wave_max(m);
-    if ((threadIdx.x & 63) == 0) atomicMax(slot + 1, __float_as_uint(m));
-}
-__global__ void rcscale_final_kernel(unsigned* __restrict__ slot) {
-    const float m = __uint_as_float(slot[1]);
-    float sc = RC_SCALE_MAX;
-    while (sc > 0x1p-40f && m * sc > 16384.f) sc *= 0.5f;
-    reinterpret_cast<float*>(slot)[0] = sc;
-}
-__global__ __launch_bounds__(256) void featsplit_kernel(const float* __restrict__ feat, half_t* __restrict__ fs,
-                                                        long long n8, const float* __restrict__ rc_scale) {
-    const long long i = (long long)blockIdx.x * 256 + threadIdx.x;
-    if (i >= n8) return;
-    const float RC_SCALE = *rc_scale;
-    const float4 a = *reinterpret_cast<const float4*>(feat + i * 8), b = *reinterpret_cast<const float4*>(feat + i * 8 + 4);
-    const float x[8] = {a.x, a.y, a.z, a.w, b.x, b.y, b.z, b.w};
-    h8 hi, lo;
-#pragma unroll
-    for (int e = 0; e < 8; ++e) {
-        const float xs = x[e] * RC_SCALE;
-        hi[e] = (half_t)xs;
-        lo[e] = (half_t)(xs - (float)hi[e]);
-    }
-    const long long chunk = i >> 2;
-    const int piece = (int)(i & 3);
-    *reinterpret_cast<h8*>(fs + chunk * 64 + piece * 8) = hi;
-    *reinterpret_cast<h8*>(fs + chunk * 64 + 32 + piece * 8) = lo;
+        if (SPLIT) {
+            const float x[8] = {a.x, a.y, a.z, a.w, b.x, b.y, b.z, b.w};
+            h8 hi, lo;
+#pragma unroll
+            for (int e = 0; e < 8; ++e) {
+                const float xs = x[e] * RC_SCALE;
+                hi[e] = (half_t)xs;
+                lo[e] = (half_t)(xs - (float)hi[e]);
+            }
+            half_t* line = fs + (rc * C + (k & ~31)) * 2 + (k & 31);
+            *reinterpret_cast<h8*>(line) = hi;
+            *reinterpret_cast<h8*>(line + 32) = lo;
+        }
+    }
 }
 
 __global__ __launch_bounds__(256) void src16_kernel(const float* __restrict__ emb, const int32_t* __restrict__ src_row,
@@ -1881,8 +1878,7 @@
     DTK_REQUIRE(g->C % CK == 0, "dtk_make_feat_f16: C=%d must be a multiple of %d for the MFMA path", g->C, CK);
     const int HWp = hw_pad(g->ph, g->pw);
     const long long cells = (long long)g->T * HWp;
-    DTK_LAUNCH("feat16", feat16_kernel, dim3(dtk_cdiv(cells, 4)), dim3(256), 0, dtk_stream(stream), feat, norms,
-               reinterpret_cast<half_t*>(feat_f16), g->T, g->ph, g->pw, pw_pad(g->pw), g->C);
+    half_t* f16 = reinterpret_cast<half_t*>(feat_f16);
     unsigned* slot = reinterpret_cast<unsigned*>(reinterpret_cast<unsigned char*>(feat_f16) + rc_scale_offset(g));
     DTK_HIP(dtk_zero_async(slot, 256, dtk_stream(stream)));
     {
@@ -1892,10 +1888,12 @@
         DTK_LAUNCH("rcscale", rcscale_final_kernel, dim3(1), dim3(1), 0, dtk_stream(stream), slot);
     }
     if (has_split_planes(g)) {
-        const long long n8 = (long long)g->T * g->ph * g->pw * g->C / 8;
-        DTK_LAUNCH("featsplit", featsplit_kernel, dim3(dtk_cdiv(n8, 256)), dim3(256), 0, dtk_stream(stream), feat,
-                   reinterpret_cast<half_t*>(reinterpret_cast<unsigned char*>(feat_f16) + split_planes_offset(g)), n8,
-                   reinterpret_cast<const float*>(slot));
+        DTK_LAUNCH("feat16_split", feat16_kernel<true>, dim3(dtk_cdiv(cells, 4)), dim3(256), 0, dtk_stream(stream), feat, norms, f16,
+                   reinterpret_cast<half_t*>(reinterpret_cast<unsigned char*>(feat_f16) + split_planes_offset(g)),
+                   reinterpret_cast<const float*>(slot), g->T, g->ph, g->pw, pw_pad(g->pw), g->C);
+    } else {
+        DTK_LAUNCH("feat16", feat16_kernel<false>, dim3(dtk_cdiv(cells, 4)), dim3(256), 0, dtk_stream(stream), feat, norms, f16,
+                   (half_t*)nullptr, (const float*)nullptr, g->T, g->ph, g->pw, pw_pad(g->pw), g->C);
     }
     return DTK_OK;
 }
diff --git a/dino_tracker_amd/csrc/vit.hip b/dino_tracker_amd/csrc/vit.hip
--- a/dino_tracker_amd/csrc/vit.hip
+++ b/dino_tracker_amd/csrc/vit.hip
@@ -220,9 +220,21 @@
     }
 }
 
-__global__ __launch_bounds__(256) void zero_kernel(uint4* __restrict__ p, long long n16) {
-    const long long i = (long long)blockIdx.x * 256 + threadIdx.x;
-    if (i < n16) p[i] = make_uint4(0, 0, 0, 0);
+__global__ __launch_bounds__(256) void zero_pad_kernel(unsigned short* __restrict__ q, unsigned short* __restrict__ k,
+                                                       unsigned short* __restrict__ vt, int S, int Sp) {
+    const size_t fh = blockIdx.x;
+    const int pad = Sp - S;
+    uint4* q4 = reinterpret_cast<uint4*>(q + (fh * Sp + S) * 64);
+    uint4* k4 = reinterpret_cast<uint4*>(k + (fh * Sp + S) * 64);
+    for (int i = threadIdx.x; i < pad * 8; i += 256) {
+        q4[i] = make_uint4(0, 0, 0, 0);
+        k4[i] = make_uint4(0, 0, 0, 0);
+    }
+    unsigned short* v = vt + fh * 64 * Sp + S;
+    for (int i = threadIdx.x; i < pad * 64; i += 256) {
+        const int r = i / pad, c = i - r * pad;
+        v[(size_t)r * Sp + c] = 0;
+    }
 }
 
 template <typename T>
@@ -476,13 +488,12 @@
     const bool scan_all = ovf && (m->flags & DTK_VIT_CHECK_RANGE);
     int* const epi_ovf = IsF16<T>::value ? ovf : nullptr;
     const int S = p.S, Sp = p.Sp;
-    {
-        const long long n16 = (long long)((p.ao - p.q) / 16);
-        DTK_LAUNCH("vit_zero", zero_kernel, dim3(dtk_cdiv(n16, 256)), dim3(256), 0, st, reinterpret_cast<uint4*>(q), n16);
-        if (p.split) {
-            const long long m16 = (long long)((p.ao_lo - p.q_lo) / 16);
-            DTK_LAUNCH("vit_zero", zero_kernel, dim3(dtk_cdiv(m16, 256)), dim3(256), 0, st, reinterpret_cast<uint4*>(q_lo), m16);
-        }
+    if (Sp > S) {
+        static_assert(sizeof(T) == 2, "zero_pad_kernel clears 2-byte operands");
+        auto u16 = [](T* t) { return reinterpret_cast<unsigned short*>(t); };
+        const unsigned fh = (unsigned)p.FB * m->heads;
+        DTK_LAUNCH("vit_zero", zero_pad_kernel, dim3(fh), dim3(256), 0, st, u16(q), u16(k), u16(vt), S, Sp);
+        if (p.split) DTK_LAUNCH("vit_zero", zero_pad_kernel, dim3(fh), dim3(256), 0, st, u16(q_lo), u16(k_lo), u16(vt_lo), S, Sp);
     }
     for (int f0 = 0; f0 < nframes; f0 += p.FB) {
         const int nf = (nframes - f0) < p.FB ? (nframes - f0) : p.FB;
diff --git a/dino_tracker_amd/ops.py b/dino_tracker_amd/ops.py
--- a/dino_tracker_amd/ops.py
+++ b/dino_tracker_amd/ops.py
@@ -369,9 +369,13 @@
               cs: torch.Tensor, anchor_th: float, cos_th: float, needed_only: bool = False) -> torch.Tensor:
     N, T = cs.shape
     occ = torch.empty((N, T), dtype=torch.uint8, device=cs.device)
-    fn = lib().dtk_occlusion_needed if needed_only else lib().dtk_occlusion
-    check(fn(_p(green, torch.float32), _p(pair_off, torch.int32), _p(pair_frame, torch.int32), _p(traj, torch.float32),
-             _p(cs, torch.float32), float(anchor_th), float(cos_th), _p(occ), N, T, _stream()))
+    args = (_p(green, torch.float32), _p(pair_off, torch.int32), _p(pair_frame, torch.int32), _p(traj, torch.float32),
+            _p(cs, torch.float32), float(anchor_th), float(cos_th), _p(occ))
+    if needed_only:
+        med = torch.empty(max(N * T, 1), dtype=torch.float32, device=cs.device)
+        check(lib().dtk_occlusion_needed(*args, _p(med), N, T, _stream()))
+    else:
+        check(lib().dtk_occlusion(*args, N, T, _stream()))
     return occ.bool()
 
 
diff --git a/include/dtk.h b/include/dtk.h
--- a/include/dtk.h
+++ b/include/dtk.h
@@ -245,7 +245,8 @@
                   const float* cs, float anchor_th, float cos_th, uint8_t* occ, int N, int T, void* stream);
 
 int dtk_occlusion_needed(const float* green, const int32_t* pair_off, const int32_t* pair_frame, const float* traj,
-                         const float* cs, float anchor_th, float cos_th, uint8_t* occ, int N, int T, void* stream);
+                         const float* cs, float anchor_th, float cos_th, uint8_t* occ, float* med_scratch, int N, int T,
+                         void* stream);
 
 int dtk_tapvid_counts(const float* pred_tracks, const uint8_t* pred_occluded, const float* gt_tracks,
                       const uint8_t* gt_occluded, const int32_t* query_frame, float pred_scale_x, float pred_scale_y,
```

Measured after the change: 532,400 query-points*frames/s (median of 6 runs). No clear change (+0.9%).
